# p3achyjr/p3achygo

Measured on AMD Instinct MI355X. Metric: self-play positions/sec at 1/8 MI355X, b12c256btl3 19x19 n=32, higher is better.
Workload: dtype f16; 1 GPU; b12c256btl3 random-init, self-play: C++ host (Gumbel MCTS n=32, default k<=5, selected k=5) -> p3hip_run over batches of 1024 leaf positions -> results back to the search; one step = one round = one engine batch of each of the 8 game groups = 8192 positions; batch_per_gpu=1024, concurrent_games_per_gpu=8192, game_groups_per_gpu=8, lanes_per_group=1, ladder_node_budget=0, parallelism=games sharded x1, no collective

## Files before the change

include/p3hip.h:

```cpp
#ifndef P3HIP_H_
#define P3HIP_H_

#include <stddef.h>
#include <stdint.h>

#ifdef __cplusplus
extern "C" {
#endif

#define P3HIP_BOARD_LEN 19
#define P3HIP_NUM_LOCS 361
#define P3HIP_NUM_MOVES 362
#define P3HIP_NUM_LAST_MOVES 5
#define P3HIP_NUM_VALUE_LOGITS 2
#define P3HIP_NUM_SCORE_LOGITS 800
#define P3HIP_NUM_PLANES 15
#define P3HIP_NUM_SCALARS 8

#define P3HIP_KIND_HIP 5

typedef struct p3hip_loc {
  int32_t i;
  int32_t j;
} p3hip_loc;
// ... 57 lines not shown
#define P3HIP_CONV_SET \
  "conv: C a multiple of 32 with 64 <= C <= 512; btl (1-3 inner layers) and nbt blocks with C_b a multiple of 16, " \
  "32 <= C_b <= C; classic blocks of two 3x3 convs (C_b ignored); broadcast blocks at any interval >= 2"

p3hip_engine* p3hip_create(const char* weights_path, int batch_size, int version,
                           int device_ordinal, uint32_t flags);
p3hip_engine* p3hip_create_rows(const char* weights_path, int batch_size, int version, int device_ordinal,
                                uint32_t flags, int symmetry_rows);
const char* p3hip_create_error(void);
void p3hip_destroy(p3hip_engine* e);

int p3hip_kind(const p3hip_engine* e);
const char* p3hip_path(const p3hip_engine* e);
int p3hip_batch_size(const p3hip_engine* e);

int p3hip_load_slot(p3hip_engine* e, int slot, const p3hip_features* f);
int p3hip_run(p3hip_engine* e);
int p3hip_get_slot(p3hip_engine* e, int slot, p3hip_result* out);
int p3hip_get_ownership(p3hip_engine* e, int slot, float out[P3HIP_NUM_LOCS]);
const char* p3hip_last_error(const p3hip_engine* e);

int p3hip_cache_enable(p3hip_engine* e, int log2_entries);
int p3hip_load_slot_keyed(p3hip_engine* e, int slot, const p3hip_features* f, uint64_t key_lo, uint64_t key_hi,
                          int symmetry);
int p3hip_get_slot_keyed(p3hip_engine* e, int slot, p3hip_result* out, int* symmetry, int* from_cache);
int p3hip_cache_stats(const p3hip_engine* e, uint64_t out[4]);

int p3hip_int8_calibrate(p3hip_engine* e);
int p3hip_int8_scales(const p3hip_engine* e, float* out, int n);
int p3hip_int8_set_scales(p3hip_engine* e, const float* scales, int n);

int p3hip_set_symmetries(p3hip_engine* e, uint32_t mask);
void p3hip_symmetry_maps(uint16_t fwd[8][361], uint16_t inv[8][361]);

int p3hip_set_slot_symmetries(p3hip_engine* e, int slot, uint32_t mask);
int p3hip_debug_symmetry_rows(const uint8_t* masks, int n, int rows, int* first, int* total);

#define P3HIP_AUX_LEN 837
int p3hip_get_aux(p3hip_engine* e, int slot, float out[P3HIP_AUX_LEN]);

typedef struct p3hip_labels {
  float policy[P3HIP_NUM_MOVES];
  float score_margin;
  int32_t did_win;
} p3hip_labels;
#define P3HIP_NUM_SCORE_TERMS 6
int p3hip_load_labels(p3hip_engine* e, int slot, const p3hip_labels* labels);
int p3hip_score(p3hip_engine* e, double sums[P3HIP_NUM_SCORE_TERMS], int* n_scored);
int p3hip_get_score(p3hip_engine* e, int slot, float terms[P3HIP_NUM_SCORE_TERMS]);
int p3hip_debug_score_rows(p3hip_engine* e, const float* move_probs, const float* value_probs, const float* score_probs,
                           const p3hip_labels* labels, int n, float* terms, double sums[P3HIP_NUM_SCORE_TERMS]);

typedef struct p3hip_targets {
  float policy[P3HIP_NUM_MOVES];
  float policy_aux_dist[P3HIP_NUM_MOVES];
  float own[P3HIP_NUM_LOCS];
  float mcts_value_dist[51];
  float score_margin, q6, q16, q50, q6_score, q16_score, q50_score;
  int32_t policy_aux;
  int32_t has_pi_aux_dist, has_mcts_value_dist;
} p3hip_targets;
#define P3HIP_NUM_LOSS_TERMS 19
int p3hip_load_targets(p3hip_engine* e, int slot, const p3hip_targets* targets);
int p3hip_loss(p3hip_engine* e, double sums[P3HIP_NUM_LOSS_TERMS], int* n);
int p3hip_get_loss(p3hip_engine* e, int slot, float terms[P3HIP_NUM_LOSS_TERMS]);
int p3hip_debug_loss_rows(p3hip_engine* e, const float* raw, const float* aux, const p3hip_targets* targets, int n,
                          float* terms, double sums[P3HIP_NUM_LOSS_TERMS]);


int p3hip_forward_resident(p3hip_engine* e, int n_positions);
int p3hip_upload(p3hip_engine* e);
int p3hip_sync(p3hip_engine* e);
#define P3HIP_RAW_LEN 1889
int p3hip_get_raw(p3hip_engine* e, int slot, float* out);
double p3hip_time_trunk_kernel(p3hip_engine* e, int n_positions, int iters,
                               double* flops_per_launch, const char** kernel_name);
const char* p3hip_debug_plan(const char* weights_path, uint32_t flags, int* n_q, uint64_t* digest);
int p3hip_debug_split(int npos, int kw, int cout, int n_cu, int* strips, int* tile);
long p3hip_debug_pack_sconv(const float* w, int taps, int cin, int cout, int cin_pad, int cout_pad, uint16_t* out, long n);
long p3hip_debug_pack_wconv(const float* w, int cin, int cout, int cin_pad, int cout_pad, uint16_t* out, long n);
int p3hip_debug_wconv_grid(int npos, int cout, int n_cu, int* grid, long* units, long unit, long* tile0, int* ntiles, int* cout0);
int p3hip_debug_tfm_split(int npos, int heads, int n_cu, int* parts, int* tokens);
int p3hip_debug_edge_split(int npos, int c_pad, int n_cu, int* stem, int* dense, int* heads);
int p3hip_graph_state(const p3hip_engine* e);
int p3hip_graph_stats(const p3hip_engine* e, uint64_t out[5]);
int p3hip_debug_graph_table(const int* npos, const int* total, int n, int capacity, int* action, int* evicted);
int p3hip_blockw_stamps(p3hip_engine* e, unsigned long long* out, int n);
int p3hip_debug_x(p3hip_engine* e, float* out, int n_positions);
int p3hip_debug_act_i8(p3hip_engine* e, int8_t* out, int n_positions);
int p3hip_debug_tfm(p3hip_engine* e, int which, float* out, int n_positions);
int p3hip_debug_poison(p3hip_engine* e, int byte);
const char* p3hip_debug_poison_table(void);
void p3hip_flops_per_position(const p3hip_engine* e, double* total, double* conv3x3);
void p3hip_rope_table(double* cos_out, double* sin_out);
int p3hip_rope_table_dim(int head_dim, double* cos_out, double* sin_out);

#ifdef __cplusplus
}
#endif
#endif
```

p3achygo_amd/csrc/engine.cpp:

```cpp
#include <hip/hip_runtime.h>
#include <chrono>

#include <cmath>
#include <cstdio>
#include <cstdlib>
#include <cstring>
#include <unordered_set>
#include <string>
#include <vector>

#include "engine.h"
#include "block_i8.h"
#include "conv_any.h"
#include "conv_f32.h"
#include "conv_split.h"
#include "conv_wino.h"
#include "edge_split.h"
#include "lconv_i8.h"
#include "loss.h"
#include "transformer.h"
#include "transformer_f32.h"
#include "transformer_split.h"

using namespace eng;

namespace {

thread_local std::string g_create_error;

unsigned char* upload_buffer(p3hip_engine* e) { return e->any_sym() ? e->d_sfeats : e->d_feats; }

bool upload(p3hip_engine* e, int n) {
  return e->check(hipMemcpyAsync(upload_buffer(e), e->feats_identity ? e->h_feats : e->h_feats_compact,
                                 (size_t)n * kFeatBytes, hipMemcpyHostToDevice, e->stream), "H2D features");
}

bool download(p3hip_engine* e, int n, const float* res) {
  const size_t rec = p3::kResultFloats * 4;
  return e->check(res ? hipMemcpyAsync(e->h_out, res, n * rec, hipMemcpyDeviceToHost, e->stream)
                      : hipMemcpy2DAsync(e->h_out, rec, e->d_out, p3::kOutStride * 4, rec, n, hipMemcpyDeviceToHost, e->stream),
                  "D2H results");
}

void free_cache(p3hip_engine::DeviceCache& c) {
  hipFree(c.d_tkeys); hipFree(c.d_tmeta); hipFree(c.d_tvals); hipFree(c.d_keys); hipFree(c.d_hit); hipFree(c.d_victim);
  hipFree(c.d_lists); hipFree(c.d_sym); hipFree(c.d_feats2);
  if (c.h_keys) hipHostFree(c.h_keys);
  if (c.h_hit) hipHostFree(c.h_hit);
  if (c.h_victim) hipHostFree(c.h_victim);
  if (c.h_lists) hipHostFree(c.h_lists);
  if (c.h_sym) hipHostFree(c.h_sym);
  delete[] c.h_slot_keys;
  c = p3hip_engine::DeviceCache{};
}

int read_acts(p3hip_engine* e, const _Float16* buf, size_t first, size_t n, float* out) {
  hipStreamSynchronize(e->stream);
  if (is_f32(e->trunk_path()))
    return hipMemcpy(out, (const float*)buf + first, n * 4, hipMemcpyDeviceToHost) == hipSuccess ? 0 : 2;
  std::vector<_Float16> h(n);
  if (hipMemcpy(h.data(), buf + first, n * 2, hipMemcpyDeviceToHost) != hipSuccess) return 2;
  for (size_t i = 0; i < n; ++i) out[i] = (float)h[i];
  return 0;
}

size_t act_elems(const p3hip_engine* e, size_t channels) { return (size_t)e->rows * channels * kNLoc; }
size_t x_bytes(const p3hip_engine* e) { return act_elems(e, e->wf.C) * act_bytes(e->trunk_path()); }
size_t t_bytes(const p3hip_engine* e) {
  const size_t C = e->wf.C;
  const size_t Ct = (e->wf.btype == 0 || e->wf.btype == 1) ? std::max<size_t>(C, 2 * (size_t)e->wf.Cb) : C;
  return act_elems(e, Ct) * act_bytes(e->trunk_path());
}
size_t s_bytes(const p3hip_engine* e) { return act_elems(e, e->wf.Cb) * 2; }
size_t qkv_bytes(const p3hip_engine* e) {
  return 3 * (size_t)e->rows * p3::kTfmLPad * (size_t)e->wf.model_C * act_bytes(e->trunk_path());
}
size_t hp_bytes(const p3hip_engine* e) { return (size_t)e->rows * 96 * kNLoc * 4; }
size_t pool_bytes(const p3hip_engine* e) { return (size_t)e->rows * p3::kHeadsPoolFloats * 4; }
size_t out_bytes(const p3hip_engine* e) { return (size_t)e->batch * p3::kOutStride * 4; }
size_t cout_bytes(const p3hip_engine* e) { return (size_t)e->rows * p3::kOutStride * 4; }
size_t res_bytes(const p3hip_engine* e) { return (size_t)e->batch * p3::kResultFloats * 4; }
size_t aux_bytes(const p3hip_engine* e) { return (size_t)e->rows * p3::kAuxStride * 4; }
size_t feats_bytes(const p3hip_engine* e) { return (size_t)e->rows * kFeatBytes; }
size_t slot_feats_bytes(const p3hip_engine* e) { return (size_t)e->batch * kFeatBytes; }
size_t symtab_bytes(const p3hip_engine* e) { return (size_t)e->batch * 5; }
size_t quant_bytes(const p3hip_engine* e) { return (size_t)e->plan.n_q * 4; }
size_t arena_bytes(const p3hip_engine* e) { return e->arena_bytes; }
size_t cache_entries(const p3hip_engine* e) { return (size_t)e->cache.mask + 1; }
size_t batch_words(const p3hip_engine* e) { return (size_t)e->batch * 4; }

bool poison_qkv_tokens(p3hip_engine* e, int byte) {
  const size_t eb = act_bytes(e->trunk_path()), D = (size_t)e->plan.choice.tfm_D;
  const size_t heads = (size_t)e->plan.choice.tfm_heads;
  return e->check(hipMemset2DAsync(e->d_qkv, p3::kTfmLPad * D * eb, byte, (size_t)kNLoc * D * eb, 3 * (size_t)e->rows * heads, e->stream),
                  "poison q, k, v");
}

enum class BufClass { Poisoned, State, Index, ZeroedOnce };

const char* class_name(BufClass c) {
  switch (c) {
    case BufClass::Poisoned: return "poisoned";
    case BufClass::State: return "state";
    case BufClass::Index: return "index";
    case BufClass::ZeroedOnce: return "zeroed-once";
  }
  return "";
}

struct DeviceBuffer {
  const char* name;
  void* (*ptr)(const p3hip_engine*);
  size_t (*bytes)(const p3hip_engine*);
  BufClass cls;
  const char* zero_range = "";
  bool (*poison_rest)(p3hip_engine*, int) = nullptr;
};

#define P3_BUF(member) #member, [](const p3hip_engine* e) -> void* { return (void*)e->member; }
#define P3_BYTES(expr) [](const p3hip_engine* e) -> size_t { return expr; }

const DeviceBuffer kDeviceBuffers[] = {
    {P3_BUF(d_x), x_bytes, BufClass::Poisoned},
    {P3_BUF(d_t), t_bytes, BufClass::Poisoned},
    {P3_BUF(d_u), x_bytes, BufClass::Poisoned},
    {P3_BUF(d_s), s_bytes, BufClass::Poisoned},
    {P3_BUF(d_qkv), qkv_bytes, BufClass::ZeroedOnce, "token rows 361..383 of every head of q, k and v", poison_qkv_tokens},
    {P3_BUF(d_hp), hp_bytes, BufClass::Poisoned},
    {P3_BUF(d_pool), pool_bytes, BufClass::Poisoned},
    {P3_BUF(d_cout), cout_bytes, BufClass::Poisoned},
    {P3_BUF(d_out), out_bytes, BufClass::Poisoned},
    {P3_BUF(d_res), res_bytes, BufClass::Poisoned},
    {P3_BUF(d_aux), aux_bytes, BufClass::Poisoned},
    {P3_BUF(scoring.d_terms), P3_BYTES(batch_words(e) * P3HIP_NUM_SCORE_TERMS), BufClass::Poisoned},
    {P3_BUF(scoring.d_sums), P3_BYTES(P3HIP_NUM_SCORE_TERMS * sizeof(double)), BufClass::Poisoned},
    {P3_BUF(loss.d_terms), P3_BYTES(batch_words(e) * P3HIP_NUM_LOSS_TERMS), BufClass::Poisoned},
    {P3_BUF(loss.d_sums), P3_BYTES(P3HIP_NUM_LOSS_TERMS * sizeof(double)), BufClass::Poisoned},
    {P3_BUF(d_arena), arena_bytes, BufClass::State},
    {P3_BUF(d_amax), quant_bytes, BufClass::State},
    {P3_BUF(d_ascale), quant_bytes, BufClass::State},
    {P3_BUF(cache.d_tkeys), P3_BYTES(cache_entries(e) * 16), BufClass::State},
    {P3_BUF(cache.d_tmeta), P3_BYTES(cache_entries(e) * 4), BufClass::State},
    {P3_BUF(cache.d_tvals), P3_BYTES(cache_entries(e) * p3::kOutStride * 4), BufClass::State},
    {P3_BUF(scoring.d_labels), P3_BYTES((size_t)e->batch * sizeof(p3hip_labels)), BufClass::State},
    {P3_BUF(loss.d_targets), P3_BYTES(batch_words(e) * p3::kTgtStride), BufClass::State},
    {P3_BUF(d_bw_stamps), P3_BYTES((size_t)8 * 16 * 4 * 24 * 8), BufClass::State},
#ifdef P3_DIAG
    {P3_BUF(d_stamps), P3_BYTES((size_t)p3::kStampWgs * 8 * p3::kStampSections * p3::kStampSlots * 8), BufClass::State},
    {P3_BUF(d_spans), P3_BYTES((size_t)p3::kSpanWgs * p3::kSpanSlots * 8), BufClass::State},
#else
    {"d_stamps", [](const p3hip_engine*) -> void* { return nullptr; }, P3_BYTES(0), BufClass::State},
    {"d_spans", [](const p3hip_engine*) -> void* { return nullptr; }, P3_BYTES(0), BufClass::State},
#endif
    {P3_BUF(d_feats), feats_bytes, BufClass::Index},
    {P3_BUF(d_sfeats), slot_feats_bytes, BufClass::Index},
    {P3_BUF(d_symtab), symtab_bytes, BufClass::Index},
    {P3_BUF(cache.d_keys), P3_BYTES((size_t)e->batch * sizeof(p3::CacheKey)), BufClass::Index},
    {P3_BUF(cache.d_hit), batch_words, BufClass::Index},
    {P3_BUF(cache.d_victim), batch_words, BufClass::Index},
    {P3_BUF(cache.d_lists), P3_BYTES(5 * batch_words(e)), BufClass::Index},
    {P3_BUF(cache.d_sym), batch_words, BufClass::Index},
    {P3_BUF(cache.d_feats2), slot_feats_bytes, BufClass::Index},
    {P3_BUF(scoring.d_rows), batch_words, BufClass::Index},
    {P3_BUF(loss.d_rows), batch_words, BufClass::Index},
};

#undef P3_BUF
#undef P3_BYTES

}

extern "C" {

const char* p3hip_create_error(void) { return g_create_error.c_str(); }
int p3hip_graph_state(const p3hip_engine* e) {
  return e->graph_failed ? -1 : (e->graph_exec || e->graph_table.held() > 0 ? 1 : 0);
}

int p3hip_graph_stats(const p3hip_engine* e, uint64_t out[5]) {
  for (int i = 0; i < 5; ++i) out[i] = 0;
  if (!(e->flags & (P3HIP_FLAG_LAUNCH_GRAPH | P3HIP_FLAG_LAUNCH_GRAPH_ANY))) return 1;
  if (e->graph_any()) {
    const gt::Table& t = e->graph_table;
    out[0] = (uint64_t)t.held(); out[1] = t.captures(); out[2] = t.replays(); out[3] = t.launches(); out[4] = t.evictions();
  } else {
    out[0] = e->graph_exec ? 1 : 0; out[1] = e->graph_captures; out[2] = e->graph_replays; out[3] = e->graph_launched;
  }
  return 0;
}

int p3hip_debug_graph_table(const int* npos, const int* total, int n, int capacity, int* action, int* evicted) {
  if (!npos || !total || !action || !evicted || n < 0 || capacity < gt::kMinCapacity || capacity > gt::kMaxCapacity) return 1;
  gt::Table table(capacity);
  static const char feats = 0, res = 0;
  for (int i = 0; i < n; ++i) {
    const gt::Step s = table.see(gt::Key{npos[i], total[i], &feats, &res}, i);
    action[i] = (int)s.action;
    evicted[i] = (int)s.evicted_tag;
  }
  return 0;
}

p3hip_engine* p3hip_create(const char* weights_path, int batch_size, int version,
                           int device_ordinal, uint32_t flags) {
  return p3hip_create_rows(weights_path, batch_size, version, device_ordinal, flags, 0);
}

p3hip_engine* p3hip_create_rows(const char* weights_path, int batch_size, int version,
                                int device_ordinal, uint32_t flags, int symmetry_rows) {
  g_create_error.clear();
  if (version != 1) { g_create_error = "only model version 1 (15 planes + 8 scalars) is supported"; return nullptr; }
  if (batch_size < 1 || batch_size > (1 << 16)) { g_create_error = "bad batch size"; return nullptr; }
  const bool sym = (flags & P3HIP_FLAG_SYMMETRY_AVG) != 0;
  const bool sym_slot = (flags & P3HIP_FLAG_SYMMETRY_SLOT) != 0;
  if (sym_slot && sym) {
    g_create_error = "P3HIP_FLAG_SYMMETRY_SLOT cannot be combined with P3HIP_FLAG_SYMMETRY_AVG: a slot's symmetries come "
                     "either from the engine's mask or from its own";
    return nullptr;
  }
  if (sym_slot && (flags & P3HIP_FLAG_AUX)) {
    g_create_error = "P3HIP_FLAG_AUX cannot be combined with P3HIP_FLAG_SYMMETRY_SLOT: the aux record holds tanh, absolute "
// ... 13 lines not shown
                       std::to_string(batch_size) + " .. 8 x batch size " + std::to_string(full);
      return nullptr;
    }
    if (want > (1 << 16)) {
      g_create_error = "P3HIP_FLAG_SYMMETRY_SLOT: symmetry_rows " + std::to_string(want) +
                       " exceeds the engine's row limit of 65536 (symmetry_rows 0 means 8 x batch size)";
      return nullptr;
    }
    symmetry_rows = (int)want;
  }
  if (sym && (size_t)p3::kNumSyms * batch_size > (1u << 16)) {
    g_create_error = "P3HIP_FLAG_SYMMETRY_AVG evaluates 8 copies of every slot: 8 x batch size " +
                     std::to_string(batch_size) + " exceeds the engine's row limit of 65536 (batch size at most 8192)";
    return nullptr;
  }
  if (sym && (flags & P3HIP_FLAG_AUX)) {
    g_create_error = "P3HIP_FLAG_AUX cannot be combined with P3HIP_FLAG_SYMMETRY_AVG: the aux record holds tanh, absolute "
                     "value and softmax outputs, and their average over symmetries is nothing the reference defines";
    return nullptr;
  }
  p3hip_engine* e = new p3hip_engine();
  e->path = weights_path;
  e->batch = batch_size;
  e->device = device_ordinal;
  e->flags = flags;
  e->opt = Options::from_env();
  if (e->graph_any()) {
    e->graph_table = gt::Table(e->opt.graph_cache, e->opt.graph_min_seen);
    e->graph_slots.resize((size_t)e->opt.graph_cache);
  }
  e->sym = sym;
  e->sym_slot = sym_slot;
  e->rows = sym ? p3::kNumSyms * batch_size : sym_slot ? symmetry_rows : batch_size;
  auto fail = [&](const std::string& m) {
    g_create_error = m;
    p3hip_destroy(e);
    return (p3hip_engine*)nullptr;
  };
  if (!e->wf.load(weights_path, e->err)) return fail(e->err);
  Arena ar;
  if (!build_plan(e->wf, flags, e->opt, e->plan, ar, e->err)) return fail(e->err);
  int ndev = 0;
  if (hipGetDeviceCount(&ndev) != hipSuccess || ndev <= device_ordinal)
    return fail("no HIP device " + std::to_string(device_ordinal) + " (the HIP engine has no CPU fallback)");
  if (!e->check(hipSetDevice(device_ordinal), "hipSetDevice")) return fail(e->err);
  hipDeviceProp_t prop;
  if (!e->check(hipGetDeviceProperties(&prop, device_ordinal), "hipGetDeviceProperties")) return fail(e->err);
  if (std::string(prop.gcnArchName).rfind("gfx950", 0) != 0)
    return fail(std::string("device is ") + prop.gcnArchName + ", this engine is built for gfx950 only");
  e->n_cu = prop.multiProcessorCount;
  const size_t B = batch_size;
  const bool copies = sym || sym_slot;
  const Path path = e->trunk_path();
  e->arena_bytes = ar.host.size();
  bool ok = e->check(hipStreamCreateWithFlags(&e->stream, hipStreamNonBlocking), "hipStreamCreate") &&
            e->check(hipMalloc((void**)&e->d_arena, arena_bytes(e)), "hipMalloc arena") &&
            e->check(hipMemcpyAsync(e->d_arena, ar.host.data(), ar.host.size(), hipMemcpyHostToDevice, e->stream), "upload weights") &&
            e->check(hipHostMalloc((void**)&e->h_feats, B * kFeatBytes, hipHostMallocDefault), "hipHostMalloc") &&
            e->check(hipHostMalloc((void**)&e->h_feats_compact, B * kFeatBytes, hipHostMallocDefault), "hipHostMalloc") &&
            e->check(hipHostMalloc((void**)&e->h_out, B * p3::kResultFloats * 4, hipHostMallocDefault), "hipHostMalloc") &&
            e->check(hipMalloc((void**)&e->d_res, res_bytes(e)), "hipMalloc results") &&
            e->check(hipMalloc((void**)&e->d_feats, feats_bytes(e)), "hipMalloc feats") &&
            e->check(hipMalloc((void**)&e->d_x, x_bytes(e)), "hipMalloc x") &&
            e->check(hipMalloc((void**)&e->d_t, t_bytes(e)), "hipMalloc t") &&
            e->check(hipMalloc((void**)&e->d_u, x_bytes(e)), "hipMalloc u") &&
            (e->wf.btype != 1 || path == Path::F32Conv || e->check(hipMalloc((void**)&e->d_s, s_bytes(e)), "hipMalloc s")) &&
            (!is_tfm(path) || e->check(hipMalloc((void**)&e->d_qkv, qkv_bytes(e)), "hipMalloc qkv")) &&
            e->check(hipMalloc((void**)&e->d_hp, hp_bytes(e)), "hipMalloc hp") &&
            ((path != Path::Split && path != Path::TfmSplit) ||
             e->check(hipMalloc((void**)&e->d_pool, pool_bytes(e)), "hipMalloc pooled")) &&
            e->check(hipMalloc((void**)&e->d_out, out_bytes(e)), "hipMalloc out") &&
            (!copies || (e->check(hipMalloc((void**)&e->d_sfeats, slot_feats_bytes(e)), "hipMalloc symmetry upload") &&
                         e->check(hipMalloc((void**)&e->d_cout, cout_bytes(e)), "hipMalloc copy rows"))) &&
            (!sym_slot || (e->check(hipMalloc((void**)&e->d_symtab, symtab_bytes(e)), "hipMalloc symmetry table") &&
                           e->check(hipHostMalloc((void**)&e->h_symtab, B * 5, hipHostMallocDefault), "hipHostMalloc") &&
                           e->check(hipMemsetAsync(e->d_symtab, 0, symtab_bytes(e), e->stream), "hipMemset symmetry table"))) &&
            (!(flags & P3HIP_FLAG_AUX) || (e->check(hipMalloc((void**)&e->d_aux, aux_bytes(e)), "hipMalloc aux") &&
                                           e->check(hipMemsetAsync(e->d_aux, 0, aux_bytes(e), e->stream), "hipMemset aux"))) &&
            (!is_int8(path) || (e->check(hipMalloc((void**)&e->d_amax, quant_bytes(e)), "hipMalloc amax") &&
                          e->check(hipMalloc((void**)&e->d_ascale, quant_bytes(e)), "hipMalloc scales") &&
                          e->check(hipMemsetAsync(e->d_amax, 0, quant_bytes(e), e->stream), "hipMemset amax") &&
                          e->check(hipMemsetAsync(e->d_ascale, 0, quant_bytes(e), e->stream), "hipMemset scales")));
  if (!ok) return fail(e->err);
  e->h_scale.assign(e->plan.n_q, 0.0f);
  memset(e->h_feats, 0, B * kFeatBytes);
  if (!e->check(hipMemsetAsync(e->d_feats, 0, feats_bytes(e), e->stream), "hipMemset feats") ||
      (copies && !e->check(hipMemsetAsync(e->d_sfeats, 0, slot_feats_bytes(e), e->stream), "hipMemset symmetry upload")) ||
      (copies && !e->check(hipMemsetAsync(e->d_cout, 0, cout_bytes(e), e->stream), "hipMemset copy rows")) ||
      (is_tfm(path) && !e->check(hipMemsetAsync(e->d_qkv, 0, qkv_bytes(e), e->stream), "hipMemset qkv")) ||
      !e->check(hipMemsetAsync(e->d_out, 0, out_bytes(e), e->stream), "hipMemset out") ||
      !e->check(hipStreamSynchronize(e->stream), "upload sync")) return fail(e->err);
  e->heads_args.conv_a = e->d_arena + e->plan.heads_conv_a_off;
  e->heads_args.image = e->dev<float>(e->plan.heads_image_off);
  e->heads_args.V = e->wf.V;
  e->heads_args.gbn_scale = e->dev<float>(e->plan.heads_gbn.scale_off);
  e->heads_args.gbn_shift = e->dev<float>(e->plan.heads_gbn.shift_off);
  for (int k = 0; k < kNumHeadTensors; ++k) e->heads_args.*kHeadTensors[k].arg = e->dev<float>(e->plan.head_tensor_off[k]);
  if (flags & P3HIP_FLAG_AUX) {
    e->aux_args.V = e->wf.V;
    e->aux_args.gbn_scale = e->heads_args.gbn_scale; e->aux_args.gbn_shift = e->heads_args.gbn_shift;
    e->aux_args.gd_w = e->heads_args.gd_w; e->aux_args.gd_b = e->heads_args.gd_b;
    e->aux_args.oq_embed_w = e->heads_args.oq_embed_w; e->aux_args.oq_embed_b = e->heads_args.oq_embed_b;
    for (int k = 0; k < kNumAuxTensors; ++k) e->aux_args.*kAuxTensors[k].arg = e->dev<float>(e->plan.aux_tensor_off[k]);
  }
  e->slots = p3::SlotStates((int)B);
  e->slot_sym.assign(B, 0);
  e->row_sym.assign(B, 0);
  e->slot_mask.assign(B, 1);
  e->row_mask.assign(B, 1);
  e->has_labels.assign(B, 0);
  e->has_targets.assign(B, 0);
  e->load_seq.assign(B, 0);
  e->run_load_seq.assign(B, 0);
  return e;
}

void p3hip_destroy(p3hip_engine* e) {
  if (!e) return;
  if (e->stream || e->d_arena) (void)hipSetDevice(e->device);
  if (e->stream) hipStreamSynchronize(e->stream);
  hipFree(e->d_arena); hipFree(e->d_feats); hipFree(e->d_x); hipFree(e->d_t); hipFree(e->d_u); hipFree(e->d_s);
  hipFree(e->d_hp); hipFree(e->d_pool); hipFree(e->d_out); hipFree(e->d_res); hipFree(e->d_qkv);
  hipFree(e->d_sfeats); hipFree(e->d_cout); hipFree(e->d_aux); hipFree(e->d_symtab);
  if (e->h_symtab) hipHostFree(e->h_symtab);
  hipFree(e->d_bw_stamps);
  hipFree(e->d_amax); hipFree(e->d_ascale);
  if (e->bw_mod) hipModuleUnload(e->bw_mod);
  free_cache(e->cache);
  free_scoring(e);
  free_loss(e);
  if (e->h_feats) hipHostFree(e->h_feats);
  if (e->h_feats_compact) hipHostFree(e->h_feats_compact);
  if (e->h_out) hipHostFree(e->h_out);
  for (hipEvent_t ev : e->blk_ev) hipEventDestroy(ev);
  drop_graph(e);
  if (e->stream) hipStreamDestroy(e->stream);
  delete e;
}

const char* p3hip_debug_plan(const char* weights_path, uint32_t flags, int* n_q, uint64_t* digest) {
  g_create_error.clear();
  WeightFile wf;
  Plan plan;
  Arena ar;
  std::string err;
  if (!wf.load(weights_path, err) || !build_plan(wf, flags, Options::from_env(), plan, ar, err)) {
    g_create_error = err;
    return nullptr;
  }
  uint64_t h = 0;
  bool any_q = false;
  auto fold = [&](size_t off, size_t bytes) {
    for (size_t i = 0; i < bytes; ++i) h = (h ^ ar.host[off + i]) * 1099511628211ull;
  };
  for (const BlockPlan& b : plan.blocks)
    for (const LayerPlan& lp : b.layers)
      if (lp.qidx >= 0) {
        if (!any_q) h = 14695981039346656037ull;
        any_q = true;
        fold(lp.q_off, (size_t)lp.kw * lp.kw * lp.cin * lp.cout);
        fold(lp.qs_off, (size_t)lp.cout * 4);
      }
  if (n_q) *n_q = plan.n_q;
  if (digest) *digest = h;
  return path_name(plan.choice.path);
}

int p3hip_debug_split(int npos, int kw, int cout, int n_cu, int* strips, int* tile) {
  const Options opt = Options::from_env();
  if (npos < 1 || (kw != 1 && kw != 3) || cout < 64 || cout % 64 != 0 || n_cu < 1 || !strips || !tile || opt.split_bad) return 1;
  if (opt.split_s) { *strips = opt.split_s; *tile = opt.split_t; }
  else p3::sconv_split(npos, kw, cout, n_cu, strips, tile);
  return 0;
}

int p3hip_debug_edge_split(int npos, int c_pad, int n_cu, int* stem, int* dense, int* heads) {
  if (stem) *stem = 1;
  if (dense) *dense = 1;
  if (heads) *heads = 1;
  const Options opt = Options::from_env();
  if (npos < 1 || !p3::edge_width_ok(c_pad) || n_cu < 1 || !stem || !dense || !heads || opt.edge_bad) return 1;
  if (opt.edge_s) {
    if (!p3::edge_split_valid(c_pad, opt.edge_s, opt.edge_d, opt.edge_h)) return 1;
    *stem = opt.edge_s; *dense = opt.edge_d; *heads = opt.edge_h;
  } else {
    p3::edge_split(npos, c_pad, n_cu, stem, dense, heads);
  }
  return 0;
}

int p3hip_debug_tfm_split(int npos, int heads, int n_cu, int* parts, int* tokens) {
  const Options opt = Options::from_env();
  if (npos < 1 || heads < 1 || n_cu < 1 || !parts || !tokens || opt.tfm_split_bad) return 1;
  if (opt.tfm_split_s) { *parts = opt.tfm_split_s; *tokens = opt.tfm_split_t; }
  else p3::tfm_split(npos, heads, n_cu, parts, tokens);
  return 0;
}

long p3hip_debug_pack_sconv(const float* w, int taps, int cin, int cout, int cin_pad, int cout_pad, uint16_t* out, long n) {
  std::vector<_Float16> img;
  p3::pack_sconv(img, w, taps, cin, cout, cin_pad, cout_pad);
  for (long i = 0; i < n && i < (long)img.size(); ++i) memcpy(out + i, &img[i], 2);
  return (long)img.size();
}

long p3hip_debug_pack_wconv(const float* w, int cin, int cout, int cin_pad, int cout_pad, uint16_t* out, long n) {
  std::vector<_Float16> img;
  p3::pack_wconv(img, w, cin, cout, cin_pad, cout_pad);
  for (long i = 0; i < n && i < (long)img.size(); ++i) memcpy(out + i, &img[i], 2);
  return (long)img.size();
}

int p3hip_debug_wconv_grid(int npos, int cout, int n_cu, int* grid, long* units, long unit, long* tile0, int* ntiles, int* cout0) {
  if (npos < 1 || cout < 64 || cout > p3::kWinoMaxC || cout % 64 != 0 || n_cu < 1 || !grid || !units) return 1;
  *grid = p3::wconv_grid(npos, cout, n_cu);
  *units = p3::wconv_units(npos, cout);
  if (unit < 0 || unit >= *units) return (tile0 || ntiles || cout0) ? 1 : 0;
  long t0 = 0;
  int nt = 0, c0 = 0;
  p3::wconv_unit(npos, cout, unit, &t0, &nt, &c0);
  if (tile0) *tile0 = t0;
  if (ntiles) *ntiles = nt;
  if (cout0) *cout0 = c0;
  return 0;
}

int p3hip_kind(const p3hip_engine*) { return P3HIP_KIND_HIP; }
const char* p3hip_path(const p3hip_engine* e) { return e->path.c_str(); }
int p3hip_batch_size(const p3hip_engine* e) { return e->batch; }
const char* p3hip_last_error(const p3hip_engine* e) { return e->err.c_str(); }

int p3hip_load_slot(p3hip_engine* e, int slot, const p3hip_features* f) {
  if (slot < 0 || slot >= e->batch) return 1;
  memcpy(e->h_feats + (size_t)slot * kFeatBytes, f, kFeatBytes);
  e->slot_sym[slot] = 0;
  e->slot_mask[slot] = 1;
  e->has_labels[slot] = 0;
  e->has_targets[slot] = 0;
  ++e->load_seq[slot];
  if (e->cache.on) e->cache.h_slot_keys[slot] = p3::CacheKey{0, 0, 0};
  e->slots.loaded(slot);
  return 0;
}

int p3hip_load_slot_keyed(p3hip_engine* e, int slot, const p3hip_features* f, uint64_t key_lo, uint64_t key_hi, int symmetry) {
  if (slot < 0 || slot >= e->batch) return 1;
  if (symmetry < 0 || symmetry > 7) return 1;
  memcpy(e->h_feats + (size_t)slot * kFeatBytes, f, kFeatBytes);
  e->slot_sym[slot] = (unsigned char)symmetry;
  e->slot_mask[slot] = 1;
  e->has_labels[slot] = 0;
  e->has_targets[slot] = 0;
  ++e->load_seq[slot];
  if (e->cache.on) e->cache.h_slot_keys[slot] = p3::CacheKey{key_lo, key_hi, (unsigned long long)symmetry};
  e->slots.loaded(slot);
  return 0;
// ... 554 lines not shown
```

p3achygo_amd/csrc/engine.h:

```cpp
#pragma once

#include <hip/hip_runtime.h>

#include <atomic>
#include <mutex>
#include <string>
#include <vector>

#include "../../include/p3hip.h"
#include "graph_table.h"
#include "heads_aux.h"
#include "kernels.h"
#include "plan.h"
#include "slot_state.h"
#include "symmetry.h"

namespace eng {

constexpr size_t kFeatBytes = sizeof(p3hip_features);
static_assert(sizeof(p3hip_features) == 1860, "p3hip_features layout");
static_assert(sizeof(p3hip_result) == 4 * 1892, "p3hip_result layout");

struct Pass {
  const unsigned char* feats = nullptr;
  int npos = 0;
  float* out = nullptr;
  float* res = nullptr;
  int* timed = nullptr;
};

struct GraphSlot {
  hipGraph_t graph = nullptr;
  hipGraphExec_t exec = nullptr;
};

}

struct p3hip_engine {
  std::string path, err;
  int batch = 0, device = 0;
  uint32_t flags = 0;
  eng::WeightFile wf;
  eng::Options opt;
  eng::Plan plan;
  int n_cu = 256;
  int last_npos = 0;
  hipModule_t bw_mod = nullptr;
  hipFunction_t bw_fn = nullptr;
  unsigned long long* d_bw_stamps = nullptr;
  hipStream_t stream = nullptr;
  hipGraph_t graph = nullptr;
  hipGraphExec_t graph_exec = nullptr;
  bool graph_failed = false, graph_warm = false;
  eng::Pass graph_pass;
  uint64_t graph_captures = 0, graph_replays = 0, graph_launched = 0;
  gt::Table graph_table;
  std::vector<eng::GraphSlot> graph_slots;
  long graph_seq = 0;
  bool graph_any() const { return (flags & P3HIP_FLAG_LAUNCH_GRAPH_ANY) != 0; }
  std::vector<hipEvent_t> blk_ev;

  unsigned char* d_arena = nullptr;
  size_t arena_bytes = 0;
  p3::HeadsArgs heads_args{};
  bool calibrating = false, have_scales = false;
  unsigned* d_amax = nullptr;
  float* d_ascale = nullptr;
  std::vector<float> h_scale;
  bool sym = false;
  uint32_t sym_mask = 0xFF;
  int sym_k = 8;
  int sym_syms[p3::kNumSyms] = {0, 1, 2, 3, 4, 5, 6, 7};
  int rows = 0;
  unsigned char* d_sfeats = nullptr;
  float* d_cout = nullptr;
  bool sym_slot = false;
  std::vector<unsigned char> slot_mask, row_mask;
  unsigned char *h_symtab = nullptr, *d_symtab = nullptr;
  int tab_n = 0, tab_total = 0;
  const int* tab_first() const { return reinterpret_cast<const int*>(d_symtab); }
  const unsigned char* tab_mask() const { return d_symtab + (size_t)batch * 4; }
  bool any_sym() const { return sym || sym_slot; }

  unsigned char* h_feats = nullptr;
  unsigned char* h_feats_compact = nullptr;
  unsigned char* d_feats = nullptr;
  _Float16 *d_x = nullptr, *d_t = nullptr, *d_u = nullptr;
  _Float16* d_qkv = nullptr;
#ifdef P3_DIAG
  unsigned long long* d_stamps = nullptr;
  unsigned long long* d_spans = nullptr;
  int launch_index = 0;
#endif
  _Float16* d_s = nullptr;
  float* d_hp = nullptr;
  float* d_pool = nullptr;
  float* d_aux = nullptr;
  p3::HeadsAuxArgs aux_args{};
  float* d_out = nullptr;
  float* h_out = nullptr;
  float* d_res = nullptr;
  double t_h2d = 0, t_fwd = 0, t_d2h = 0;
  long t_runs = 0;
  bool feats_identity = false;
  p3::SlotStates slots;
  int last_n = 0;
  std::vector<unsigned char> slot_sym, row_sym;

  struct DeviceCache {
    bool on = false;
    unsigned mask = 0, run = 0;
    unsigned long long* d_tkeys = nullptr;
    unsigned* d_tmeta = nullptr;
    float* d_tvals = nullptr;
    p3::CacheKey* h_slot_keys = nullptr;
    p3::CacheKey *h_keys = nullptr, *d_keys = nullptr;
    int *h_hit = nullptr, *d_hit = nullptr, *h_victim = nullptr, *d_victim = nullptr;
    int *h_lists = nullptr, *d_lists = nullptr;
    unsigned *h_sym = nullptr, *d_sym = nullptr;
    unsigned char* d_feats2 = nullptr;
    std::vector<int> out_row;
    std::vector<unsigned char> was_hit;
    unsigned long long lookups = 0, hits = 0, inserts = 0;
  } cache;
  struct Scoring {
    std::mutex mu;
    std::atomic<bool> ready{false};
    p3hip_labels *h_slot = nullptr, *h_dense = nullptr, *d_labels = nullptr;
    int *h_rows = nullptr, *d_rows = nullptr;
    float *h_terms = nullptr, *d_terms = nullptr;
    double *h_sums = nullptr, *d_sums = nullptr;
    std::vector<int> entry_of_slot;
    long scored_run = -1;
  } scoring;
  std::vector<unsigned char> has_labels;
  struct Loss {
    std::mutex mu;
    std::atomic<bool> ready{false};
    float *h_slot = nullptr, *h_dense = nullptr, *d_targets = nullptr;
    int *h_rows = nullptr, *d_rows = nullptr;
    float *h_terms = nullptr, *d_terms = nullptr;
    double *h_sums = nullptr, *d_sums = nullptr;
    std::vector<int> entry_of_slot;
    long loss_run = -1;
  } loss;
  std::vector<unsigned char> has_targets;
// ... 38 lines not shown
```

p3achygo_amd/csrc/forward.cpp:

```cpp
#include <algorithm>
#include <cstdlib>
#include <cstring>
#include <string>

#include "block_i8.h"
#include "conv_any.h"
#include "conv_f32.h"
#include "conv_split.h"
#include "conv_wino.h"
#include "edge_split.h"
#include "engine.h"
#include "lconv_conv3.h"
#include "lconv_i8.h"
#include "transformer.h"
#include "transformer_f32.h"
#include "transformer_split.h"

namespace eng {
namespace {

int grid_for(const p3hip_engine* e, int npos, int npos_per_wg) {
  int wgs = (npos + npos_per_wg - 1) / npos_per_wg;
  return wgs < e->n_cu ? wgs : e->n_cu;
}
// ... 118 lines not shown
  if (kind != 0 && kind != 1) return 0;
  int n = 1;
  while (e->opt.fuse && n < p3::kMaxFuse && first + n < blocks.size() && blocks[first + n].kind == kind) ++n;
  return n;
}

}
}

extern "C" const unsigned char p3_blockw_hsaco[];
extern "C" const unsigned char p3_blockw_hsaco_end[];

namespace eng {
namespace {

struct BlockwArgs {
  const void* x; const void* ws; const void* prm;
  int npos, nblk, nwg, pad;
  void* stamps;
  unsigned long long pad2[2];
};
static_assert(sizeof(BlockwArgs) == 64, "kernarg layout of k_blockw");

bool load_blockw(p3hip_engine* e) {
  if (e->bw_fn) return true;
  if (!e->check(hipModuleLoadData(&e->bw_mod, p3_blockw_hsaco), "hipModuleLoadData k_blockw")) return false;
  const std::string name = "k_blockw_L" + std::to_string(e->wf.inner) + (e->opt.blockw_diag ? "_diag" : "");
  if (!e->check(hipModuleGetFunction(&e->bw_fn, e->bw_mod, name.c_str()), "hipModuleGetFunction k_blockw")) return false;
  if (e->opt.blockw_diag) {
    constexpr size_t bytes = 8 * 16 * 4 * 24 * 8;
    if (!e->check(hipMalloc((void**)&e->d_bw_stamps, bytes), "hipMalloc stamps") ||
        !e->check(hipMemsetAsync(e->d_bw_stamps, 0, bytes, e->stream), "hipMemset stamps")) return false;
  }
  return true;
}

bool launch_blockw(p3hip_engine* e, const BlockwRun& run, int npos) {
  if (!load_blockw(e)) return false;
  BlockwArgs a{};
  a.x = e->d_x;
  a.ws = e->d_arena + run.stream_off;
  a.prm = e->d_arena + run.prm_off;
  a.npos = npos;
  a.nblk = run.nblk;
  a.nwg = npos < e->n_cu ? npos : e->n_cu;
  a.stamps = e->d_bw_stamps;
  size_t size = sizeof a;
  void* cfg[] = {HIP_LAUNCH_PARAM_BUFFER_POINTER, &a, HIP_LAUNCH_PARAM_BUFFER_SIZE, &size, HIP_LAUNCH_PARAM_END};
  return e->check(hipModuleLaunchKernel(e->bw_fn, a.nwg, 1, 1, 256, 1, 1, 0, e->stream, nullptr, cfg), "launch k_blockw");
}

template <class Launch>
bool timed_launch(p3hip_engine* e, int* timed, Launch&& launch) {
  const bool on = timed && 2 * *timed + 1 < (int)e->blk_ev.size();
  if (on) hipEventRecord(e->blk_ev[2 * *timed], e->stream);
  if (!launch()) return false;
  if (on) hipEventRecord(e->blk_ev[2 * (*timed)++ + 1], e->stream);
  return true;
}


hipError_t launch_conv1x1(const p3hip_engine* e, int which, const p3::Conv1x1Args& a) {
  return runs_conv_any(e->plan.choice) ? p3::launch_conv1x1_any(e->wf.C, which, a, e->n_cu, e->stream)
                                    : p3::launch_conv1x1(e->wf.C, which, a, e->n_cu, e->stream);
}

bool enqueue_stem(p3hip_engine* e, const Pass& p) {
  const Plan& pl = e->plan;
  const int C = e->wf.C;
  if (is_f32(e->trunk_path())) {
    const p3::InitF32Args a{p.feats, (float*)e->d_x, p.npos, C, e->dev<float>(pl.init_w_off), e->dev<float>(pl.game_w_off),
                            e->dev<float>(pl.game_b_off)};
    return e->check(p3::launch_init_f32(a, e->n_cu, e->stream), "launch k_init_f32");
  }
  p3::InitArgs a{};
  a.feats = p.feats; a.x = e->d_x; a.npos = p.npos;
  a.wstream = e->d_arena + pl.init_w_off; a.nms_total = pl.init_nms;
  a.game_w = e->dev<float>(pl.game_w_off); a.game_b = e->dev<float>(pl.game_b_off);
  if (e->trunk_path() == Path::Split || e->trunk_path() == Path::TfmSplit) {
    int stem = 1, dense = 1, heads = 1;
    edge_split_of(e, p.npos, &stem, &dense, &heads);
    if (stem > 1) return e->check(p3::launch_init_split(C, a, stem, e->n_cu, e->stream), "launch k_init_split");
  }
  return e->check(runs_conv_any(e->plan.choice) ? p3::launch_init_any(C, a, grid_for(e, p.npos, 1), e->stream)
                                             : p3::launch_init(C, a, grid_for(e, p.npos, 1), e->stream), "launch k_init");
}

bool enqueue_tfm_block(p3hip_engine* e, const Pass& p, const BlockPlan& bp) {
  const int d = e->wf.model_C, D = e->plan.choice.tfm_D, npos = p.npos;
  hipStream_t s = e->stream;
  const size_t per = (size_t)e->rows * p3::kTfmLPad * d;
  _Float16 *q = e->d_qkv, *k = q + per, *v = k + per, *o = e->d_t;
  p3::TfmQkvArgs a{e->d_x, q, k, v, npos, e->dev<float>(bp.tfm.rms_in), e->d_arena + bp.tfm.wqkv,
                   e->dev<float>(e->plan.rope_cos_off), e->dev<float>(e->plan.rope_sin_off)};
  int parts = 1, tokens = 64;
  if (e->trunk_path() == Path::TfmSplit) tfm_split_of(e, npos, &parts, &tokens);
  if (!e->check(p3::launch_tfm_qkv_split(d, D, a, tokens, s), "launch k_tfm_qkv")) return false;
  const p3::TfmAttnArgs b{q, k, v, o, npos, e->plan.choice.tfm_heads};
  if (!timed_launch(e, p.timed, [&] { return e->check(p3::launch_tfm_attn_split(D, b, parts, s), "launch k_tfm_attn"); }))
    return false;
  const p3::TfmFfnArgs f{o, e->d_x, npos, e->d_arena + bp.tfm.wo, e->dev<float>(bp.tfm.rms_out),
                         e->d_arena + bp.tfm.wgu, e->d_arena + bp.tfm.wdown};
  return e->check(p3::launch_tfm_ffn_split(d, f, tokens, s), "launch k_tfm_ffn");
}

bool enqueue_tfm_block_f32(p3hip_engine* e, const Pass& p, const BlockPlan& bp) {
  const int d = e->wf.model_C, D = e->plan.choice.tfm_D, npos = p.npos;
  hipStream_t s = e->stream;
  const size_t per = (size_t)e->rows * p3::kTfmLPad * d;
  float *x = (float*)e->d_x, *q = (float*)e->d_qkv, *k = q + per, *v = k + per, *o = (float*)e->d_t;
  const p3::TfmQkvF32Args a{x, q, k, v, npos, d, D, e->dev<float>(bp.tfm.rms_in), e->dev<float>(bp.tfm.wqkv),
                            e->dev<float>(e->plan.rope_cos_off), e->dev<float>(e->plan.rope_sin_off)};
  if (!e->check(p3::launch_tfm_qkv_f32(a, s), "launch k_tfm_qkv_f32")) return false;
  const p3::TfmAttnF32Args b{q, k, v, o, npos, e->plan.choice.tfm_heads};
  if (!timed_launch(e, p.timed, [&] { return e->check(p3::launch_tfm_attn_f32(D, b, s), "launch k_tfm_attn_f32"); }))
    return false;
  const p3::TfmFfnF32Args f{o, x, npos, d, e->dev<float>(bp.tfm.wo), e->dev<float>(bp.tfm.rms_out),
                            e->dev<float>(bp.tfm.wgu), e->dev<float>(bp.tfm.wdown)};
  return e->check(p3::launch_tfm_ffn_f32(f, s), "launch k_tfm_ffn_f32");
}

template <class T>
struct Regions {
  T* buf[5];
  explicit Regions(const p3hip_engine* e) {
    const size_t half = (size_t)e->rows * e->wf.Cb * kNLoc;
    T *x = (T*)e->d_x, *t = (T*)e->d_t, *u = (T*)e->d_u;
    buf[0] = x; buf[1] = t; buf[2] = t + half; buf[3] = u; buf[4] = u + half;
  }
};

template <class Args, class T>
void fill_layer(const p3hip_engine* e, Args& a, const LayerPlan& lp, const Regions<T>& r, int npos) {
  a.in = r.buf[lp.in_buf]; a.out = r.buf[lp.out_buf]; a.npos = npos;
  a.out2 = lp.out2_buf >= 0 ? reinterpret_cast<decltype(a.out2)>(r.buf[lp.out2_buf]) : nullptr;
  a.pre = lp.pre; a.act = lp.act; a.res = lp.res; a.dual = lp.dual;
  if (a.pre) { a.scale_in = e->dev<float>(lp.pre_bn.scale_off); a.shift_in = e->dev<float>(lp.pre_bn.shift_off); }
  if (a.act == 1 || a.dual) { a.scale_out = e->dev<float>(lp.out_bn.scale_off); a.shift_out = e->dev<float>(lp.out_bn.shift_off); }
}

bool launch_layer(p3hip_engine* e, const Pass& p, const LayerPlan& lp, const char* what = nullptr) {
  const LayerKernel k = layer_kernel(e, lp.kw);
  const bool conv3 = e->trunk_path() == Path::Int8Conv3;
  switch (k) {
    case LayerKernel::LconvF32: {
      p3::LConvF32Args a{};
      fill_layer(e, a, lp, Regions<float>(e), p.npos);
      a.cin = lp.cin; a.cout = lp.cout; a.w = e->dev<float>(lp.w_off);
      return e->check(p3::launch_lconv_f32(lp.kw, a, e->n_cu, e->stream), what ? what : "launch k_lconv_f32");
    }
    case LayerKernel::Sconv: {
      p3::SConvArgs a{};
      fill_layer(e, a, lp, Regions<_Float16>(e), p.npos);
      a.cin = lp.cin; a.cout = lp.cout; a.w = e->d_arena + lp.w_off;
      if (e->opt.split_s) { a.strips = e->opt.split_s; a.tile = e->opt.split_t; }
      else p3::sconv_split(a.npos, lp.kw, a.cout, e->n_cu, &a.strips, &a.tile);
      return e->check(p3::launch_sconv(lp.kw, a, e->n_cu, e->stream), what ? what : "launch k_sconv");
    }
    case LayerKernel::Wconv: {
      p3::WConvArgs a{};
      fill_layer(e, a, lp, Regions<_Float16>(e), p.npos);
      a.cin = lp.cin; a.cout = lp.cout; a.w = e->d_arena + lp.wino_off;
      return e->check(p3::launch_wconv(a, e->n_cu, e->stream), what ? what : "launch k_wconv");
    }
    case LayerKernel::LconvI8:
    case LayerKernel::LconvI8Any: {
// ... 80 lines not shown
  p3::Conv1x1Args c1{};
  c1.in = e->d_u; c1.out16 = e->d_x; c1.npos = npos;
  c1.wstream = e->d_arena + last.w_off; c1.nms_total = last.nms;
  return bp.last_fused || e->check(launch_conv1x1(e, 1, c1), "launch conv_last");
}

bool enqueue_block_i8(p3hip_engine* e, const Pass& p, const BlockPlan& bp) {
  p3::BlockI8Args a{};
  a.x = e->d_x; a.npos = p.npos; a.inner = e->wf.inner;
  a.act_scale = e->d_ascale; a.q0 = bp.layers[0].qidx;
  for (size_t j = 0; j < bp.layers.size(); ++j) {
    const LayerPlan& lp = bp.layers[j];
    a.w[j] = e->dev<int8_t>(lp.q_off); a.w_scale[j] = e->dev<float>(lp.qs_off);
    const FoldedBN& bn = j == 0 ? lp.pre_bn : bp.layers[j - 1].out_bn;
    a.scale[j] = e->dev<float>(bn.scale_off); a.shift[j] = e->dev<float>(bn.shift_off);
  }
  auto launch = [&] { return e->check(p3::launch_block_i8(e->wf.C, a, e->n_cu, e->stream), "launch k_block_i8"); };
  return timed_launch(e, p.timed, launch);
}

bool enqueue_blockw_run(p3hip_engine* e, const Pass& p, size_t bi, int* covered) {
  const int r = e->plan.blocks[bi].bw_run;
  if (r < 0) { e->err = "internal error: no k_blockw run starts at this block"; return false; }
  const BlockwRun& run = e->plan.bw_runs[r];
  *covered = run.nblk;
  return timed_launch(e, p.timed, [&] { return launch_blockw(e, run, p.npos); });
}

bool enqueue_fused_run(p3hip_engine* e, const Pass& p, size_t bi, int* covered) {
  p3::BlockArgs a;
  *covered = joined_launch(e, bi, p.npos, &a);
  if (*covered == 0) {
    *covered = fused_run(e, bi);
    a = block_args(e, bi, *covered, p.npos);
  }
#ifdef P3_DIAG
  {
    static const int which = getenv("P3DIAG_LAUNCH") ? atoi(getenv("P3DIAG_LAUNCH")) : 1;
    constexpr size_t bytes = (size_t)p3::kStampWgs * 8 * p3::kStampSections * p3::kStampSlots * 8;
    if (!e->d_stamps && hipMalloc((void**)&e->d_stamps, bytes) == hipSuccess) hipMemset(e->d_stamps, 0, bytes);
    constexpr size_t span_bytes = (size_t)p3::kSpanWgs * p3::kSpanSlots * 8;
    if (!e->d_spans && hipMalloc((void**)&e->d_spans, span_bytes) == hipSuccess) hipMemset(e->d_spans, 0, span_bytes);
    static const int which_run = getenv("P3DIAG_RUN") ? atoi(getenv("P3DIAG_RUN")) : 1;
    const int idx = (a.nruns > 1) ? 0 : which;
    a.stamp_run = (a.nruns > 1) ? which_run : 0;
    a.spans = (e->launch_index == idx) ? e->d_spans : nullptr;
    a.stamps = (e->launch_index++ == idx) ? e->d_stamps : nullptr;
  }
#endif
  const int kind = e->plan.blocks[bi].kind;
  auto launch = [&] {
    return e->check(p3::launch_block(e->wf.C, kind, e->wf.inner, e->opt.c128_wg8, a, e->n_cu, e->stream), "launch k_block");
  };
  return timed_launch(e, p.timed, launch);
}

bool enqueue_heads(p3hip_engine* e, const Pass& p) {
  const int C = e->wf.C;
  if (is_f32(e->trunk_path())) {
    p3::LConvF32Args hc{};
    hc.in = (const float*)e->d_x; hc.out = e->d_hp; hc.npos = p.npos; hc.cin = C; hc.cout = 128; hc.hp = 1;
    hc.w = e->dev<float>(e->plan.heads_w_off);
    if (!e->check(p3::launch_lconv_f32(1, hc, e->n_cu, e->stream), "launch head convs (fp32)")) return false;
  } else if (!e->plan.choice.heads_fused) {
    p3::Conv1x1Args c{};
    c.in = e->d_x; c.out32 = e->d_hp; c.npos = p.npos;
    c.wstream = e->d_arena + e->plan.heads_w_off; c.nms_total = e->plan.heads_nms;
    if (!e->check(launch_conv1x1(e, 2, c), "launch head convs")) return false;
  }
  const bool aux = (e->flags & P3HIP_FLAG_AUX) != 0;
  if (aux && e->plan.choice.heads_fused) {
    p3::Conv1x1Args c{};
    c.in = e->d_x; c.out32 = e->d_hp; c.npos = p.npos;
    c.wstream = e->d_arena + e->plan.heads_w_off; c.nms_total = e->plan.heads_nms;
    if (!e->check(launch_conv1x1(e, 2, c), "launch head convs (aux)")) return false;
  }
  p3::HeadsArgs h = e->heads_args;
  h.x = e->d_x; h.hp = e->d_hp; h.out = p.out; h.res = p.res; h.npos = p.npos;
  int hparts = 1;
  if (!e->plan.choice.heads_fused && (e->trunk_path() == Path::Split || e->trunk_path() == Path::TfmSplit)) {
    int stem = 1, dense = 1;
    edge_split_of(e, p.npos, &stem, &dense, &hparts);
  }
  if (!(e->plan.choice.heads_fused ? e->check(p3::launch_headsx(C, h, e->n_cu, e->stream), "launch k_headsx")
        : hparts > 1               ? e->check(p3::launch_heads_split(h, e->d_pool, hparts, e->stream), "launch k_heads_pool / points / softmax")
                                   : e->check(p3::launch_heads(h, p.npos, e->stream), "launch k_heads"))) return false;
  if (!aux) return true;
  p3::HeadsAuxArgs x = e->aux_args;
  x.hp = e->d_hp; x.aux = e->d_aux; x.npos = p.npos;
  return e->check(p3::launch_heads_aux(x, e->n_cu, e->stream), "launch k_heads_aux");
}

}

void tfm_split_of(const p3hip_engine* e, int npos, int* parts, int* tokens) {
  if (e->opt.tfm_split_s) { *parts = e->opt.tfm_split_s; *tokens = e->opt.tfm_split_t; }
  else p3::tfm_split(npos, e->plan.choice.tfm_heads, e->n_cu, parts, tokens);
}

void edge_split_of(const p3hip_engine* e, int npos, int* stem, int* dense, int* heads) {
  if (e->opt.edge_s) { *stem = e->opt.edge_s; *dense = e->opt.edge_d; *heads = e->opt.edge_h; }
  else p3::edge_split(npos, e->wf.C, e->n_cu, stem, dense, heads);
}

LayerKernel layer_kernel(const p3hip_engine* e, int kw) {
  const Path path = e->trunk_path();
  if (path == Path::Int8Conv3) {
    const bool any = e->plan.choice.any_width;
    if (kw == 3 && !e->calibrating) return any ? LayerKernel::LconvI8Any : LayerKernel::LconvI8;
    return any ? LayerKernel::LconvAny : LayerKernel::Lconv;
  }
  if (path == Path::Winograd3) return kw == 3 ? LayerKernel::Wconv : e->plan.choice.any_width ? LayerKernel::LconvAny : LayerKernel::Lconv;
  if (path == Path::F32Conv) return LayerKernel::LconvF32;
  if (path == Path::Split) return LayerKernel::Sconv;
  if (is_int8(path) && !e->calibrating) return path == Path::Int8Any ? LayerKernel::LconvI8Any : LayerKernel::LconvI8;
  return runs_conv_any(e->plan.choice) || path == Path::Int8Fused128 ? LayerKernel::LconvAny : LayerKernel::Lconv;
}

const char* layer_kernel_name(LayerKernel k, int kw, int cin, int cout) {
  switch (k) {
    case LayerKernel::Lconv: return cin == 192 ? "k_lconv<3,192,192>" : "k_lconv<3,64,64>";
    case LayerKernel::LconvAny: return p3::lconv_any_kernel_name(kw);
    case LayerKernel::LconvI8: return p3::lconv_i8_kernel_name(kw, cin, cout);
    case LayerKernel::LconvI8Any: return p3::lconv_i8_any_kernel_name(kw);
    case LayerKernel::LconvF32: return p3::lconv_f32_kernel_name(kw);
    case LayerKernel::Sconv: return p3::sconv_kernel_name(kw);
    case LayerKernel::Wconv: return p3::wconv_kernel_name();
  }
  return nullptr;
}

bool enqueue_forward(p3hip_engine* e, const Pass& p) {
  const Path path = e->trunk_path();
  const std::vector<BlockPlan>& blocks = e->plan.blocks;
  if (!enqueue_stem(e, p)) return false;
#ifdef P3_DIAG
  e->launch_index = 0;
#endif
  const int stop_block = e->opt.stop_block;
  e->last_npos = p.npos;
  for (size_t bi = 0; bi < blocks.size(); ++bi) {
    if (stop_block >= 0 && (int)bi >= stop_block) return true;
    const BlockPlan& bp = blocks[bi];
    int covered = 1;
    bool ok = false;
    switch (bp.kind) {
      case 5:
        ok = path == Path::TfmF32 ? enqueue_tfm_block_f32(e, p, bp) : enqueue_tfm_block(e, p, bp);
        break;
      case 3:
        ok = path == Path::F32Conv || path == Path::Split ? enqueue_broadcast_block_layers(e, p, bp) : enqueue_broadcast_block(e, p, bp);
        break;
      case 4:
        ok = is_int8_fused(path) && !e->calibrating ? enqueue_block_i8(e, p, bp) : enqueue_layerwise_block(e, p, bp);
        break;
      default:
        ok = path == Path::Blockw ? enqueue_blockw_run(e, p, bi, &covered) : enqueue_fused_run(e, p, bi, &covered);
    }
    if (!ok) return false;
    bi += covered - 1;
  }
  if (stop_block == (int)blocks.size()) return true;
  return enqueue_heads(e, p);
}

bool stage_sym_table(p3hip_engine* e, const unsigned char* masks, int n) {
  const size_t B = (size_t)e->batch;
// ... 148 lines not shown
```

p3achygo_amd/csrc/heads_dense_phase.inc:

```
  if (t < H) {
    float s = hl[L::gd_b + t];
#pragma unroll 8
    for (int k = 0; k < 2 * H; ++k) s += sc[L::gp + k] * hl[L::gd_w + k * H + t];
    sc[L::gbias + t] = s;
  } else if (t >= 64 && t < 64 + V) {
    const int o = t - 64;
    float s = hl[L::oq_embed_b + o], gm = hl[L::gamma_pre_b + o], b = hl[L::score_pre_b + o];
#pragma unroll 8
    for (int k = 0; k < 2 * H; ++k) {
      const float x = sc[L::vp + k];
      s += x * hl[L::oq_embed_w + k * V + o];
      gm += x * hl[L::gamma_pre_w + k * V + o];
      b += x * hl[L::score_pre_w + k * V + o];
    }
    sc[L::emb + o] = mish_f(s);
    sc[L::gpre + o] = mish_f(gm);
    sc[L::base + o] = b;
  } else if (t == 192) {
    float s0 = pass_b0, so = opt_pass_b;
#pragma unroll 8
    for (int k = 0; k < 2 * H; ++k) {
      s0 += sc[L::gp + k] * hl[L::pass_w + k * 2];
      so += sc[L::gp + k] * hl[L::opt_pass_w + k];
    }
    sc[L::pi + 361] = s0 - 3.0f;
    sc[L::opt + 361] = so - 3.0f;
  }
  __syncthreads();
  if (t < 14) {
    float s = hl[L::oq_out_b + t];
#pragma unroll 8
    for (int k = 0; k < V; ++k) s += sc[L::emb + k] * hl[L::oq_out_w + k * 14 + t];
    if (t < 2) sc[L::misc + t] = s;
    if (live) {
      if (t < 2) out[kOffOutcomeLogits + t] = s;
      if (t == 5) {
        out[kOffErr2] = 4.0f / (1.0f + __expf(-s));
        if (res) res[kOffErr2] = out[kOffErr2];
      }
    }
  } else if (t == 64) {
    float s = gamma_out_b;
#pragma unroll 8
    for (int k = 0; k < V; ++k) s += sc[L::gpre + k] * hl[L::gamma_out_w + k];
    if (live) out[kOffGamma] = s;
    const float sp = s > 20.0f ? s : log1pf(__expf(s));
    sc[L::misc + 2] = fminf(sp, 10.0f);
  }
```

p3achygo_amd/csrc/kernels.h:

```cpp
#pragma once
#include <hip/hip_runtime.h>
#include <stdint.h>

namespace p3 {

constexpr int kOffMoveLogits = 0;
constexpr int kOffMoveProbs = 362;
constexpr int kOffValueProbs = 724;
constexpr int kOffScoreProbs = 726;
constexpr int kOffOptProbs = 1526;
constexpr int kOffErr2 = 1888;
constexpr int kResultFloats = 1889;
constexpr int kOffOptLogits = 1889;
constexpr int kOffOutcomeLogits = 2251;
constexpr int kOffScoreLogits = 2253;
constexpr int kOffOwnership = 3053;
constexpr int kOffGamma = 3414;
constexpr int kOutStride = 3416;

constexpr int kMaxBlockLayers = 8;

constexpr int kMaxFuse = 6;
constexpr int kMaxRuns = 4, kMaxLaunchBlocks = 12;
struct BlockParams {
// ... 29 lines not shown
  int stamp_run;
  unsigned long long* spans;
#endif
};
#ifdef P3_DIAG
constexpr int kStampWgs = 8, kStampSections = 8, kStampSlots = 32, kSpanWgs = 512, kSpanSlots = 16;
#endif

struct InitArgs {
  const void* feats;
  _Float16* x;
  int npos;
  const void* wstream;
  int nms_total;
  const float* game_w;
  const float* game_b;
};

struct Conv1x1Args {
  const _Float16* in;
  _Float16* out16;
  float* out32;
  int npos;
  const void* wstream;
  int nms_total;
  const float* scale;
  const float* shift;
};

struct LConvArgs {
  const _Float16* in;
  _Float16* out;
  _Float16* out2;
  int npos;
  const void* wstream;
  int nms_total;
  int pre, act, res, dual;
  const float *scale_in, *shift_in;
  const float *scale_out, *shift_out;
  int pair_split;
};

struct BDenseArgs {
  const _Float16* t;
  _Float16* u;
  int npos;
  const void* wstream;
  int nms_total;
  const float* bias;
  const float* scale;
  const float* shift;
};

constexpr int heads_image_floats(int H, int V) {
  return 2 * H * H + 2 * H * V + 2 * H * V + (2 * H + 1) * V + V * 14 + V + V + 4 * H + 2 * H + 2 * H + H + H + H + H + H + V + V + V + 16;
}

struct HeadsArgs {
  const float* hp;
  const _Float16* x;
  const void* conv_a;
  const float* image;
  float* out;
  float* res;
  int npos;
  int V;
  const float *gbn_scale, *gbn_shift;
  const float *gd_w, *gd_b;
  const float *moves_w;
  const float *pass_w, *pass_b;
  const float *opt_moves_w;
  const float *opt_pass_w, *opt_pass_b;
  const float *oq_embed_w, *oq_embed_b;
  const float *oq_out_w, *oq_out_b;
  const float *own_w;
  const float *gamma_pre_w, *gamma_pre_b;
  const float *gamma_out_w, *gamma_out_b;
  const float *score_pre_w, *score_pre_b;
  const float *score_out_w, *score_out_b;
};

hipError_t launch_block(int C, int kind, int L, bool wg8, const BlockArgs& a, int n_cu, hipStream_t s);
int block_macro_step_bytes(int C, bool wg8);
hipError_t launch_init(int C, const InitArgs& a, int grid, hipStream_t s);
hipError_t launch_conv1x1(int C, int which, const Conv1x1Args& a, int n_cu, hipStream_t s);
hipError_t launch_bdense(int C, const BDenseArgs& a, int grid, hipStream_t s);
hipError_t launch_lconv(int kw, int cin, int cout, const LConvArgs& a, int n_cu, hipStream_t s);
hipError_t launch_heads(const HeadsArgs& a, int grid, hipStream_t s);
inline bool heads_fusable(int C, int V) { return (C == 128 || C == 256) && (V == 32 || V == 48 || V == 64); }
hipError_t launch_headsx(int C, const HeadsArgs& a, int n_cu, hipStream_t s);

constexpr int kCacheWays = 8;
struct CacheKey { unsigned long long lo, hi, sym; };
struct CacheArgs {
  const CacheKey* keys;
  int n;
  unsigned long long* tkeys;
  unsigned* tmeta;
  float* tvals;
  unsigned mask;
  unsigned run;
  int* hit;
  int* victim;
  const int* rows;
  const int* src;
  const int* idx;
  int m;
  int out_row0;
  float* out;
  unsigned* out_sym;
  const unsigned char* feats_in;
  unsigned char* feats_out;
};
hipError_t launch_cache_probe(const CacheArgs& a, hipStream_t s);
hipError_t launch_cache_gather(const CacheArgs& a, hipStream_t s);
hipError_t launch_cache_fill(const CacheArgs& a, hipStream_t s);
hipError_t launch_cache_insert(const CacheArgs& a, hipStream_t s);
const char* block_kernel_name(int C, int kind, int L);

}
```

p3achygo_amd/csrc/kernels.hip:

```cpp
#include "kernels.h"

#include <hip/hip_runtime.h>

#include "conv_core.h"
#include "conv16.h"
#include "launch_util.h"
#include "layer_kernels.h"

namespace p3 {

#ifdef P3_DIAG
#define P3_STAMP(section, k)                                                                              \
  do {                                                                                                    \
    if (a.stamps && blockIdx.x < kStampWgs && npos_done == 1 && run == a.stamp_run && (section) < kStampSections && (threadIdx.x & 63) == 0) \
      a.stamps[((blockIdx.x * 8 + (threadIdx.x >> 6)) * kStampSections + (section)) * kStampSlots + (k)] = \
          __builtin_amdgcn_s_memtime();                                                                   \
  } while (0)
#define P3_SPAN(k)                                                                        \
  do {                                                                                    \
    if (a.spans && blockIdx.x < kSpanWgs && threadIdx.x == 0 && (k) < 8) {                \
      a.spans[blockIdx.x * kSpanSlots + (k)] = __builtin_amdgcn_s_memtime();              \
      a.spans[blockIdx.x * kSpanSlots + 8 + (k)] = __builtin_amdgcn_s_memrealtime();      \
    }                                                                                     \
  } while (0)
// ... 202 lines not shown
            EpiOut16<NT> A0;
            residual_addr16<G, CB, NT>(xin, C, pos0, a.npos, 0);
            residual_load16<NT>(xin, a.x);
            activate_loaded16<G, CB, NT>(A0, xin, a.tail_scale[run], a.tail_shift[run], 0);
            residual_addr16<G, CB, NT>(xin, C, pos0, a.npos, CB);
            residual_load16<NT>(xin, a.x);
            stash16<NT>(A1, xin);
            epilogue_write16<G, CB, NT>(smem, A0, 0);
            ring_note_inflight(ring, 12);
          }
          acc16_zero<NT>(acc);
          P3_STAMP(7, 16 * half + 1);
          conv_segment16<G, CB, 1, 1, true>(ring, smem, acc);
          P3_STAMP(7, 16 * half + 2);
          if (half == 1) activate_stashed16<G, CB, NT>(A1, a.tail_scale[run], a.tail_shift[run], CB);
          lds_barrier();
          epilogue_write16<G, CB, NT>(smem, A1, 0);
          P3_STAMP(7, 16 * half + 3);
          conv_segment16<G, CB, 1, 1, true>(ring, smem, acc);
          P3_STAMP(7, 16 * half + 4);
          lds_barrier();
          epilogue_tt16<G, CB, kTtStride, NT>(smem, acc);
          bdense_stage_params(FixedW<C>{}, prm, a.dense_bias[run], a.dense_scale[run], a.dense_shift[run]);
          P3_STAMP(7, 16 * half + 5);
          bdense_passes(FixedW<C>{}, ring, smem, prm, prm + 384, prm + 384 + C, uout, pos0, half, kTtChannels);
          P3_STAMP(7, 16 * half + 6);
          if (half == 1 && run + 1 < nruns) asm volatile("s_waitcnt vmcnt(0)" ::: "memory");
          lds_barrier();
          act_zero<G>(smem);
          lds_barrier();
          P3_STAMP(7, 16 * half + 7);
        }
        blk0 += nblk;
        continue;
      }
    }
    if (tail) {
      f32x4 acc[4][NT];
      ResRegs16<NT> tr;
      P3_STAMP(7, 0);
      ring_note_inflight(ring, 24);
      acc16_zero<NT>(acc);
      P3_STAMP(7, 1);
      conv_segment16<G, CB, 1, 1>(ring, smem, acc);
      P3_STAMP(7, 2);
      lds_barrier();
      epilogue_write16<G, CB, NT>(smem, A1, 0);
      P3_STAMP(7, 4);
      conv_segment16<G, CB, 1, 1>(ring, smem, acc);
      P3_STAMP(7, 5);
      residual_addr16<G, CB, NT>(tr, C, pos0, a.npos, 0);
      epilogue_store16_mish<NT>(acc, tr, a.tout);
      P3_STAMP(7, 6);
      {
        ResRegs16<NT> xin;
        residual_addr16<G, CB, NT>(xin, C, pos0, a.npos, 0);
        residual_load16<NT>(xin, a.x);
        stash16<NT>(A1, xin);
      }
      ring_note_inflight(ring, 12);
      acc16_zero<NT>(acc);
      P3_STAMP(7, 7);
      conv_segment16<G, CB, 1, 1>(ring, smem, acc);
      P3_STAMP(7, 8);
      activate_stashed16<G, CB, NT>(A1, a.tail_scale[run], a.tail_shift[run], 0);
      lds_barrier();
      epilogue_write16<G, CB, NT>(smem, A1, 0);
      P3_STAMP(7, 10);
      conv_segment16<G, CB, 1, 1>(ring, smem, acc);
      P3_STAMP(7, 11);
      lds_barrier();
      residual_addr16<G, CB, NT>(tr, C, pos0, a.npos, CB);
      epilogue_store16_mish<NT>(acc, tr, a.tout);
      P3_STAMP(7, 12);
    }
    blk0 += nblk;
    }
    P3_SPAN(2 + npos_done < 7 ? 2 + npos_done : 6);
  }
  ring_drain();
  P3_SPAN(7);
}

template <int C, int CP = 128>
__global__ void __launch_bounds__(kWG, 2) k_init(InitArgs a) {
  init_body<CP>(a, FixedW<C>{});
}

template <int CIN, int COUT, bool PRE, int EPI>
__global__ void __launch_bounds__(kWG, 2) k_conv1x1(Conv1x1Args a) {
  constexpr int CB = CIN >= 256 ? 128 : 64;
  constexpr int CP = (COUT >= 128 && CB == 128) ? 128 : 64;
  conv1x1_body<CB, CP, PRE, EPI>(a, FixedW<CIN>{}, FixedW<COUT>{});
}

template <int KW, int CIN, int COUT, bool PRE, bool ACT, bool RES, bool DUAL = false, int NW = 8>
__global__ void __launch_bounds__(NW * 64, 2) k_lconv(LConvArgs a) {
  lconv_body<KW, PRE, ACT, RES, DUAL, NW>(a, FixedW<CIN / 64>{}, FixedW<COUT / 64>{});
}

template <int C>
__global__ void __launch_bounds__(kWG, 2) k_bdense(BDenseArgs a) {
  bdense_body(a, FixedW<C>{});
}

template <int H, int V>
struct HeadsLds {
  static constexpr int gd_w = 0;
  static constexpr int oq_embed_w = gd_w + 2 * H * H;
  static constexpr int gamma_pre_w = oq_embed_w + 2 * H * V;
  static constexpr int score_pre_w = gamma_pre_w + 2 * H * V;
  static constexpr int oq_out_w = score_pre_w + (2 * H + 1) * V;
  static constexpr int gamma_out_w = oq_out_w + V * 14;
  static constexpr int score_out_w = gamma_out_w + V;
  static constexpr int pass_w = score_out_w + V;
  static constexpr int opt_pass_w = pass_w + 4 * H;
  static constexpr int moves_w = opt_pass_w + 2 * H;
  static constexpr int opt_moves_w = moves_w + 2 * H;
  static constexpr int own_w = opt_moves_w + H;
  static constexpr int gbn_scale = own_w + H;
  static constexpr int gbn_shift = gbn_scale + H;
  static constexpr int gd_b = gbn_shift + H;
  static constexpr int oq_embed_b = gd_b + H;
  static constexpr int gamma_pre_b = oq_embed_b + V;
  static constexpr int score_pre_b = gamma_pre_b + V;
  static constexpr int oq_out_b = score_pre_b + V;
  static constexpr int n_weights = oq_out_b + 16;
  static constexpr int gp = 0, vp = gp + 2 * H, gbias = vp + 2 * H, emb = gbias + H, gpre = emb + V,
                       base = gpre + V, red = base + V, misc = red + 16, logits = misc + 4,
                       pi = logits + 800, opt = pi + 364, n_scratch = opt + 364;
  static constexpr int kGroups = 4;
  static constexpr size_t bytes = (size_t)(n_weights + kGroups * n_scratch) * 4;
};

template <int H, int V>
__global__ void __launch_bounds__(1024) k_heads(HeadsArgs a) {
  static_assert(H == 32, "head channels");
  using L = HeadsLds<H, V>;
  extern __shared__ __attribute__((aligned(16))) float hl[];
  const int tid = threadIdx.x, g = tid >> 8, t = tid & 255;
  const int wid = t >> 6, lane = t & 63;
  auto stage = [&](int off, const float* __restrict__ src, int n) {
    for (int i = tid; i < n; i += 1024) hl[off + i] = src[i];
  };
  stage(L::gd_w, a.gd_w, 2 * H * H);
  stage(L::oq_embed_w, a.oq_embed_w, 2 * H * V);
  stage(L::gamma_pre_w, a.gamma_pre_w, 2 * H * V);
  stage(L::score_pre_w, a.score_pre_w, (2 * H + 1) * V);
  stage(L::oq_out_w, a.oq_out_w, V * 14);
  stage(L::gamma_out_w, a.gamma_out_w, V);
  stage(L::score_out_w, a.score_out_w, V);
  stage(L::pass_w, a.pass_w, 4 * H);
  stage(L::opt_pass_w, a.opt_pass_w, 2 * H);
  stage(L::moves_w, a.moves_w, 2 * H);
  stage(L::opt_moves_w, a.opt_moves_w, H);
  stage(L::own_w, a.own_w, H);
  stage(L::gbn_scale, a.gbn_scale, H);
  stage(L::gbn_shift, a.gbn_shift, H);
  stage(L::gd_b, a.gd_b, H);
  stage(L::oq_embed_b, a.oq_embed_b, V);
  stage(L::gamma_pre_b, a.gamma_pre_b, V);
  stage(L::score_pre_b, a.score_pre_b, V);
  stage(L::oq_out_b, a.oq_out_b, 14);
  const float pass_b0 = a.pass_b[0], opt_pass_b = a.opt_pass_b[0], gamma_out_b = a.gamma_out_b[0],
              score_out_b = a.score_out_b[0];
  float* sc = hl + L::n_weights + g * L::n_scratch;
  const float* base = sc + L::base, * w_sp = hl + L::score_pre_w + (2 * H) * V, * w_so = hl + L::score_out_w;
  __syncthreads();

  for (int pos4 = blockIdx.x * L::kGroups; pos4 < a.npos; pos4 += gridDim.x * L::kGroups) {
    const bool live = pos4 + g < a.npos;
    const int pos = live ? pos4 + g : a.npos - 1;
    const f32x4* __restrict__ hp4 = (const f32x4*)(a.hp + (size_t)pos * 3 * H * kNLoc);
    float* __restrict__ out = a.out + (size_t)pos * kOutStride;
    float* __restrict__ res = a.res ? a.res + (size_t)pos * kResultFloats : nullptr;
    static_assert(H % 4 == 0, "channel quads");
    for (int qd = wid; qd < 2 * H / 4; qd += 4) {
      const int c = 4 * qd;
      const f32x4* src = hp4 + (size_t)(H / 4 + qd) * kNLoc;
      f32x4 v[6];
#pragma unroll
      for (int k = 0; k < 6; ++k) {
        const int i = lane + 64 * k;
        v[k] = src[i < kNLoc ? i : kNLoc - 1];
      }
      const bool is_g = c < H;
      const int ch = is_g ? c : c - H;
#pragma unroll
      for (int e = 0; e < 4; ++e) {
        const float bsc = is_g ? hl[L::gbn_scale + ch + e] : 1.0f, bsh = is_g ? hl[L::gbn_shift + ch + e] : 0.0f;
        float s = 0.0f, m = -3.0e38f;
#pragma unroll
        for (int k = 0; k < 6; ++k) {
          float x = v[k][e];
          if (is_g) x = mish_f(x * bsc + bsh);
          if (lane + 64 * k < kNLoc) {
            s += x;
            m = fmaxf(m, x);
          }
        }
        s = wave_sum(s);
        m = wave_max(m);
        if (lane == 0) {
          float* dst = sc + (is_g ? L::gp : L::vp);
          dst[ch + e] = s * (1.0f / kNLoc);
          dst[H + ch + e] = m;
        }
      }
    }
    __syncthreads();
#include "heads_dense_phase.inc"
    for (int i = t; i < kNLoc; i += 256) {
      float pi = 0.0f, po = 0.0f, ow = 0.0f;
      const int z = launder(0);
#pragma unroll
      for (int c0 = 0; c0 < H; c0 += 8) {
        float pv[8], vv[8];
#pragma unroll
        for (int u = 0; u < 2; ++u) {
          const f32x4 p4 = hp4[(size_t)(c0 / 4 + u) * kNLoc + i];
          const f32x4 v4 = hp4[(size_t)(2 * H / 4 + c0 / 4 + u) * kNLoc + i];
#pragma unroll
          for (int e = 0; e < 4; ++e) {
            pv[4 * u + e] = p4[e];
            vv[4 * u + e] = v4[e];
          }
        }
#pragma unroll
        for (int c = 0; c < 8; ++c) {
          const float p = mish_f(pv[c] + sc[L::gbias + z + c0 + c]);
          pi += p * hl[L::moves_w + z + (c0 + c) * 2];
          po += p * hl[L::opt_moves_w + z + c0 + c];
          ow += vv[c] * hl[L::own_w + z + c0 + c];
        }
      }
      sc[L::pi + i] = pi;
      sc[L::opt + i] = po;
      if (live) out[kOffOwnership + i] = tanhf(ow);
    }
    __syncthreads();
    {
      const float gam = sc[L::misc + 2];
      for (int sidx = t; sidx < 800; sidx += 256) {
#include "heads_score_bin.inc"
        sc[L::logits + sidx] = gam * s;
      }
    }
    __syncthreads();
#include "heads_softmax_phase.inc"
  }
}

template <int C, int H, int V>
struct HeadsxLds {
  using L = HeadsLds<H, V>;
  static constexpr int kGroups = 2, NS = C / 32;
  static constexpr int part = L::n_weights + kGroups * L::n_scratch;
  static constexpr int n_part = kGroups * 4 * 4 * H;
  static constexpr size_t conv_off = ((size_t)(part + n_part) * 4 + 15) / 16 * 16;
  static constexpr size_t bytes = conv_off + (size_t)6 * NS * 1024;
};

template <int C, int H, int V>
__global__ void __launch_bounds__(512, 2) k_headsx(HeadsArgs a) {
  static_assert(H == 32 && C % 32 == 0, "head channels");
  using L = HeadsLds<H, V>;
  using X = HeadsxLds<C, H, V>;
  constexpr int NS = X::NS;
  extern __shared__ __attribute__((aligned(16))) float hl[];
  const int tid = threadIdx.x, g = tid >> 8, t = tid & 255;
  const int wid = t >> 6, lane = t & 63;
  const int n = lane & 15, q = lane >> 4;
  static_assert(L::n_weights == heads_image_floats(H, V) && L::n_weights % 4 == 0, "image = HeadsLds");
  {
    const f32x4* src = (const f32x4*)a.image;
    f32x4* dst = (f32x4*)hl;
    for (int i = tid; i < L::n_weights / 4; i += 512) dst[i] = src[i];
  }
  {
    const f32x4* src = (const f32x4*)a.conv_a;
    f32x4* dst = (f32x4*)((char*)hl + X::conv_off);
    for (int i = tid; i < 6 * NS * 64; i += 512) dst[i] = src[i];
  }
  const float pass_b0 = a.pass_b[0], opt_pass_b = a.opt_pass_b[0], gamma_out_b = a.gamma_out_b[0],
              score_out_b = a.score_out_b[0];
  float* sc = hl + L::n_weights + g * L::n_scratch;
  float* part = hl + X::part + g * (4 * 4 * H);
  const char* wlds = (const char*)hl + X::conv_off + lane * 16;
  __syncthreads();

  constexpr int NTILE = (kNLoc + 15) / 16;
  constexpr int TPW = (NTILE + 3) / 4;
  for (int pos2 = blockIdx.x * X::kGroups; pos2 < a.npos; pos2 += gridDim.x * X::kGroups) {
    const bool live = pos2 + g < a.npos;
    const int pos = live ? pos2 + g : a.npos - 1;
    float* __restrict__ out = a.out + (size_t)pos * kOutStride;
    float* __restrict__ res = a.res ? a.res + (size_t)pos * kResultFloats : nullptr;
    const _Float16* __restrict__ xp = a.x + (size_t)pos * C * kNLoc;
    float bsc[2][4], bsh[2][4], ownw[2][4];
#pragma unroll
    for (int u = 0; u < 2; ++u)
#pragma unroll
      for (int i = 0; i < 4; ++i) {
        bsc[u][i] = hl[L::gbn_scale + 16 * u + 4 * q + i];
        bsh[u][i] = hl[L::gbn_shift + 16 * u + 4 * q + i];
        ownw[u][i] = hl[L::own_w + 16 * u + 4 * q + i];
      }
    float gs[2][4], gm[2][4], vs[2][4], vm[2][4];
#pragma unroll
    for (int u = 0; u < 2; ++u)
#pragma unroll
      for (int i = 0; i < 4; ++i) { gs[u][i] = 0.0f; gm[u][i] = -3.0e38f; vs[u][i] = 0.0f; vm[u][i] = -3.0e38f; }
    f32x4 P[TPW][2];
    auto xload = [&](h8 (&xb)[NS], int tile) {
      int loc = tile * 16 + n;
      if (loc >= kNLoc) loc = kNLoc - 1;
      const _Float16* src = xp + ((size_t)q * kNLoc + loc) * 8;
#pragma unroll
      for (int s_ = 0; s_ < NS; ++s_) xb[s_] = *(const h8*)(src + (size_t)s_ * 4 * kNLoc * 8);
    };
    h8 xb[2][NS];
    xload(xb[0], wid);
#pragma unroll
    for (int k = 0; k < TPW; ++k) {
      const int tile = wid + 4 * k;
      if (k + 1 < TPW) xload(xb[(k + 1) & 1], (tile + 4 < NTILE) ? tile + 4 : NTILE - 1);
      f32x4 acc[6];
#pragma unroll
      for (int ct = 0; ct < 6; ++ct) acc[ct] = f32x4{0.f, 0.f, 0.f, 0.f};
#pragma unroll
      for (int s_ = 0; s_ < NS; ++s_)
#pragma unroll
        for (int ct = 0; ct < 6; ++ct)
          acc[ct] = __builtin_amdgcn_mfma_f32_16x16x32_f16(*(const h8*)(wlds + (ct * NS + s_) * 1024), xb[k & 1][s_], acc[ct], 0, 0, 0);
      const int loc = tile * 16 + n;
      const bool ok = tile < NTILE && loc < kNLoc;
      P[k][0] = acc[0];
      P[k][1] = acc[1];
      float ow = 0.0f;
#pragma unroll
      for (int u = 0; u < 2; ++u)
#pragma unroll
        for (int i = 0; i < 4; ++i) {
          const float y = mish_f(acc[2 + u][i] * bsc[u][i] + bsh[u][i]);
          const float v = acc[4 + u][i];
          if (ok) {
            gs[u][i] += y;
            gm[u][i] = fmaxf(gm[u][i], y);
            vs[u][i] += v;
            vm[u][i] = fmaxf(vm[u][i], v);
          }
          ow += v * ownw[u][i];
        }
      ow += __shfl_xor(ow, 16);
      ow += __shfl_xor(ow, 32);
      if (ok && live && q == 0) out[kOffOwnership + loc] = tanhf(ow);
    }
#pragma unroll
    for (int u = 0; u < 2; ++u)
#pragma unroll
      for (int i = 0; i < 4; ++i) {
#pragma unroll
        for (int m = 1; m < 16; m <<= 1) {
          gs[u][i] += __shfl_xor(gs[u][i], m);
          gm[u][i] = fmaxf(gm[u][i], __shfl_xor(gm[u][i], m));
          vs[u][i] += __shfl_xor(vs[u][i], m);
          vm[u][i] = fmaxf(vm[u][i], __shfl_xor(vm[u][i], m));
        }
        if (n == 0) {
          const int ch = 16 * u + 4 * q + i;
          float* pw = part + wid * (4 * H);
          pw[ch] = gs[u][i];
          pw[H + ch] = gm[u][i];
          pw[2 * H + ch] = vs[u][i];
          pw[3 * H + ch] = vm[u][i];
        }
      }
    __syncthreads();
    if (t < 4 * H) {
      const int kind = t / H, ch = t - kind * H;
      const float p0 = part[kind * H + ch], p1 = part[4 * H + kind * H + ch], p2 = part[8 * H + kind * H + ch],
                  p3 = part[12 * H + kind * H + ch];
      float* dst = sc + ((kind < 2) ? L::gp : L::vp);
      if ((kind & 1) == 0) dst[ch] = (p0 + p1 + p2 + p3) * (1.0f / kNLoc);
      else dst[H + ch] = fmaxf(fmaxf(p0, p1), fmaxf(p2, p3));
    }
    __syncthreads();
#include "heads_dense_phase.inc"
    {
      float gb[2][4], mw[2][4], omw[2][4];
#pragma unroll
      for (int u = 0; u < 2; ++u)
#pragma unroll
        for (int i = 0; i < 4; ++i) {
          const int c = 16 * u + 4 * q + i;
          gb[u][i] = sc[L::gbias + c];
          mw[u][i] = hl[L::moves_w + c * 2];
          omw[u][i] = hl[L::opt_moves_w + c];
        }
#pragma unroll
      for (int k = 0; k < TPW; ++k) {
        const int tile = wid + 4 * k;
        float pi = 0.0f, po = 0.0f;
#pragma unroll
        for (int u = 0; u < 2; ++u)
#pragma unroll
          for (int i = 0; i < 4; ++i) {
            const float pm = mish_f(P[k][u][i] + gb[u][i]);
            pi += pm * mw[u][i];
            po += pm * omw[u][i];
          }
        pi += __shfl_xor(pi, 16);
        pi += __shfl_xor(pi, 32);
        po += __shfl_xor(po, 16);
        po += __shfl_xor(po, 32);
        const int loc = tile * 16 + n;
        if (q == 0 && tile < NTILE && loc < kNLoc) {
          sc[L::pi + loc] = pi;
          sc[L::opt + loc] = po;
        }
      }
    }
    __syncthreads();
    {
      const float gam = sc[L::misc + 2];
#pragma unroll
      for (int pr = 0; pr < 2; ++pr) {
        const int s0 = t + 512 * pr, s1 = s0 + 256;
        const f32x2 sv = {0.05f * (float)(s0 - 400) + 0.025f, 0.05f * (float)(s1 - 400) + 0.025f};
        f32x2 acc = {score_out_b, score_out_b};
        const int z = launder(0);
#pragma unroll 8
        for (int k = 0; k < V; ++k) {
          const float b = sc[L::base + z + k], w = hl[L::score_pre_w + (2 * H) * V + z + k], o = hl[L::score_out_w + z + k];
          acc = __builtin_elementwise_fma(mish_f2(__builtin_elementwise_fma(sv, f32x2{w, w}, f32x2{b, b})), f32x2{o, o}, acc);
        }
        sc[L::logits + s0] = gam * acc[0];
        if (s1 < 800) sc[L::logits + s1] = gam * acc[1];
      }
    }
    __syncthreads();
#include "heads_softmax_phase.inc"
  }
}

template <int C, int CB, int KIND, int L, int NW, bool BC>
static hipError_t launch_block_bc(const BlockArgs& a, int n_cu, hipStream_t s) {
  constexpr int NPOS = NW == 8 ? 128 / CB : 1;
  using G = Geo<NPOS, CB, 3, NW, NW == 8 ? kKMS : 2, NW == 8 ? kRingDepth : kRingDepth4>;
  constexpr size_t lds = G::ACT_BYTES + ring_bytes(CB, G::KMS, G::RD);
  static AttrOnce once;
  if (hipError_t e = ensure_lds(once, k_block<C, CB, KIND, L, NW, BC>, lds); e != hipSuccess) return e;
  const int groups = (a.npos + NPOS - 1) / NPOS, cap = NW == 8 ? n_cu : 2 * n_cu;
  hipLaunchKernelGGL((k_block<C, CB, KIND, L, NW, BC>), dim3(groups < cap ? groups : cap), dim3(NW * 64), lds, s, a);
  return hipGetLastError();
}
template <int C, int CB, int KIND, int L, int NW>
static hipError_t launch_block_t(const BlockArgs& a, int n_cu, hipStream_t s) {
  if (a.head || a.tail || a.nruns > 1) return launch_block_bc<C, CB, KIND, L, NW, true>(a, n_cu, s);
  return launch_block_bc<C, CB, KIND, L, NW, false>(a, n_cu, s);
}

int block_macro_step_bytes(int C, bool wg8) { return C == 256 ? 128 * 32 * kKMS : (wg8 ? 64 * 32 * kKMS : 64 * 32 * 2); }

hipError_t launch_block(int C, int kind, int L, bool wg8, const BlockArgs& a, int n_cu, hipStream_t s) {
  if (C == 256 && kind == 0 && L == 3) return launch_block_t<256, 128, 0, 3, 8>(a, n_cu, s);
  if (C == 256 && kind == 0 && L == 2) return launch_block_t<256, 128, 0, 2, 8>(a, n_cu, s);
  if (C == 256 && kind == 0 && L == 1) return launch_block_t<256, 128, 0, 1, 8>(a, n_cu, s);
  if (C == 256 && kind == 1) return launch_block_t<256, 128, 1, 2, 8>(a, n_cu, s);
  if (C == 128 && wg8) {
    if (kind == 0 && L == 3) return launch_block_t<128, 64, 0, 3, 8>(a, n_cu, s);
    if (kind == 0 && L == 2) return launch_block_t<128, 64, 0, 2, 8>(a, n_cu, s);
    if (kind == 0 && L == 1) return launch_block_t<128, 64, 0, 1, 8>(a, n_cu, s);
    if (kind == 1) return launch_block_t<128, 64, 1, 2, 8>(a, n_cu, s);
  }
  if (C == 128 && kind == 0 && L == 3) return launch_block_t<128, 64, 0, 3, 4>(a, n_cu, s);
  if (C == 128 && kind == 0 && L == 2) return launch_block_t<128, 64, 0, 2, 4>(a, n_cu, s);
  if (C == 128 && kind == 0 && L == 1) return launch_block_t<128, 64, 0, 1, 4>(a, n_cu, s);
  if (C == 128 && kind == 1) return launch_block_t<128, 64, 1, 2, 4>(a, n_cu, s);
  return hipErrorInvalidValue;
}

template <class K>
static hipError_t set_lds(K kernel, size_t lds) {
  return hipFuncSetAttribute((const void*)kernel, hipFuncAttributeMaxDynamicSharedMemorySize, (int)lds);
}

hipError_t launch_init(int C, const InitArgs& a, int grid, hipStream_t s) {
  using G = Geo<1, 16, 5>;
  constexpr size_t lds = G::ACT_BYTES + ring_bytes(128) + 384 * 4;
  if (C == 192) {
    constexpr size_t lds64 = G::ACT_BYTES + ring_bytes(64) + 192 * 4;
    hipLaunchKernelGGL((k_init<192, 64>), dim3(grid), dim3(kWG), lds64, s, a);
  } else if (C == 384) {
    hipLaunchKernelGGL((k_init<384>), dim3(grid), dim3(kWG), lds, s, a);
  } else if (C == 256) {
    hipLaunchKernelGGL((k_init<256>), dim3(grid), dim3(kWG), lds, s, a);
  } else if (C == 128) {
    hipLaunchKernelGGL((k_init<128>), dim3(grid), dim3(kWG), lds, s, a);
  } else {
    return hipErrorInvalidValue;
  }
  return hipGetLastError();
}

template <int CIN, int COUT, bool PRE, int EPI>
static hipError_t launch_conv1x1_t(const Conv1x1Args& a, int n_cu, hipStream_t s) {
  constexpr int CB = CIN >= 256 ? 128 : 64;
  using G = Geo<128 / CB, CB, 1>;
  constexpr int CP = (COUT >= 128 && CB == 128) ? 128 : 64;
  const int grid = conv_split_grid(a.npos, 128 / CB, (COUT + CP - 1) / CP, n_cu);
  constexpr size_t lds = G::ACT_BYTES + ring_bytes(CP);
  static AttrOnce once;
  if (hipError_t e = ensure_lds(once, k_conv1x1<CIN, COUT, PRE, EPI>, lds); e != hipSuccess) return e;
  hipLaunchKernelGGL((k_conv1x1<CIN, COUT, PRE, EPI>), dim3(grid), dim3(kWG), lds, s, a);
  return hipGetLastError();
}

hipError_t launch_conv1x1(int C, int which, const Conv1x1Args& a, int grid, hipStream_t s) {
  if (C == 192) {
    if (which == 0) return launch_conv1x1_t<192, 192, true, 0>(a, grid, s);
    if (which == 1) return launch_conv1x1_t<192, 192, false, 1>(a, grid, s);
    if (which == 2) return launch_conv1x1_t<192, 96, false, 2>(a, grid, s);
  } else if (C == 384) {
    if (which == 0) return launch_conv1x1_t<384, 384, true, 0>(a, grid, s);
    if (which == 1) return launch_conv1x1_t<384, 384, false, 1>(a, grid, s);
    if (which == 2) return launch_conv1x1_t<384, 96, false, 2>(a, grid, s);
  } else if (C == 256) {
    if (which == 0) return launch_conv1x1_t<256, 256, true, 0>(a, grid, s);
    if (which == 1) return launch_conv1x1_t<256, 256, false, 1>(a, grid, s);
    if (which == 2) return launch_conv1x1_t<256, 96, false, 2>(a, grid, s);
  } else if (C == 128) {
    if (which == 0) return launch_conv1x1_t<128, 128, true, 0>(a, grid, s);
    if (which == 1) return launch_conv1x1_t<128, 128, false, 1>(a, grid, s);
    if (which == 2) return launch_conv1x1_t<128, 96, false, 2>(a, grid, s);
  }
  return hipErrorInvalidValue;
}

template <int KW, int CIN, int COUT, bool PRE, bool ACT, bool RES, bool DUAL, int NW>
static hipError_t launch_lconv_nw(const LConvArgs& a, int n_cu, hipStream_t s) {
  constexpr int NPOS = NW == 8 ? 2 : 1;
  using G = Geo<NPOS, 64, KW, NW, (NW == 4 && KW == 3) ? 2 : kKMS>;
  const int grid = conv_split_grid(a.npos, NPOS, COUT / 64, NW == 8 ? n_cu : 2 * n_cu);
  constexpr size_t lds = G::ACT_BYTES + ring_bytes(64, G::KMS);
  static_assert(NW == 8 || 2 * lds <= 160 * 1024, "two workgroups per CU");
  static AttrOnce once;
  if (hipError_t e = ensure_lds(once, k_lconv<KW, CIN, COUT, PRE, ACT, RES, DUAL, NW>, lds); e != hipSuccess) return e;
  LConvArgs b = a;
  b.nms_total = a.nms_total * (kKMS / G::KMS);
  static const bool turns = getenv("P3HIP_NO_PAIR_TURNS") == nullptr;
  b.pair_split = (NW == 4 && turns && grid > n_cu) ? n_cu : 0;
  hipLaunchKernelGGL((k_lconv<KW, CIN, COUT, PRE, ACT, RES, DUAL, NW>), dim3(grid), dim3(NW * 64), lds, s, b);
  return hipGetLastError();
}
template <int KW, int CIN, int COUT, bool PRE, bool ACT, bool RES, bool DUAL>
static hipError_t launch_lconv_t(const LConvArgs& a, int n_cu, hipStream_t s) {
  static const bool wg8 = getenv("P3HIP_LCONV_WG8") != nullptr;
  if (wg8) return launch_lconv_nw<KW, CIN, COUT, PRE, ACT, RES, DUAL, 8>(a, n_cu, s);
  return launch_lconv_nw<KW, CIN, COUT, PRE, ACT, RES, DUAL, 4>(a, n_cu, s);
}

hipError_t launch_lconv(int kw, int cin, int cout, const LConvArgs& a, int grid, hipStream_t s) {
  const int f = (a.pre ? 8 : 0) | (a.act ? 4 : 0) | (a.res ? 2 : 0) | (a.dual ? 1 : 0);
#define P3_LCONV(KW, CIN, COUT, PRE, ACT, RES, DUAL) \
  if (kw == KW && cin == CIN && cout == COUT && f == ((PRE ? 8 : 0) | (ACT ? 4 : 0) | (RES ? 2 : 0) | (DUAL ? 1 : 0))) \
    return launch_lconv_t<KW, CIN, COUT, PRE, ACT, RES, DUAL>(a, grid, s);
  P3_LCONV(1, 384, 192, true, true, false, false)
  P3_LCONV(1, 384, 192, false, true, false, false)
  P3_LCONV(1, 384, 192, true, false, false, true)
  P3_LCONV(1, 384, 192, false, false, false, true)
  P3_LCONV(3, 192, 192, false, true, false, false)
  P3_LCONV(3, 192, 192, true, true, false, false)
  P3_LCONV(3, 192, 192, false, false, true, false)
  P3_LCONV(3, 192, 192, false, false, true, true)
  P3_LCONV(1, 192, 384, false, false, true, false)
  P3_LCONV(1, 192, 384, false, false, true, true)
  P3_LCONV(1, 256, 128, true, true, false, false)
  P3_LCONV(3, 128, 128, false, true, false, false)
  P3_LCONV(1, 128, 256, false, false, true, false)
#undef P3_LCONV
  return hipErrorInvalidValue;
}

hipError_t launch_bdense(int C, const BDenseArgs& a, int grid, hipStream_t s) {
  constexpr size_t lds = 128 * kTtStride + ring_bytes(128) + (384 + 2 * 384) * 4;
  static AttrOnce once[4];
  {
    hipError_t e = C == 256 ? ensure_lds(once[0], k_bdense<256>, lds) : C == 128 ? ensure_lds(once[1], k_bdense<128>, lds)
                 : C == 384 ? ensure_lds(once[2], k_bdense<384>, lds) : C == 192 ? ensure_lds(once[3], k_bdense<192>, lds)
                 : hipErrorInvalidValue;
    if (e != hipSuccess) return e;
  }
  if (C == 192) {
    hipLaunchKernelGGL((k_bdense<192>), dim3(grid), dim3(kWG), lds, s, a);
  } else if (C == 384) {
    hipLaunchKernelGGL((k_bdense<384>), dim3(grid), dim3(kWG), lds, s, a);
  } else if (C == 256) {
    hipLaunchKernelGGL((k_bdense<256>), dim3(grid), dim3(kWG), lds, s, a);
  } else if (C == 128) {
    hipLaunchKernelGGL((k_bdense<128>), dim3(grid), dim3(kWG), lds, s, a);
  } else {
    return hipErrorInvalidValue;
  }
  return hipGetLastError();
}

template <int V>
static hipError_t launch_heads_t(const HeadsArgs& a, hipStream_t s) {
  using L = HeadsLds<32, V>;
  static AttrOnce once;
  if (hipError_t e = ensure_lds(once, k_heads<32, V>, L::bytes); e != hipSuccess) return e;
  const int grid = (a.npos + L::kGroups - 1) / L::kGroups;
  hipLaunchKernelGGL((k_heads<32, V>), dim3(grid), dim3(1024), L::bytes, s, a);
  return hipGetLastError();
}

template <int C, int V>
static hipError_t launch_headsx_t(const HeadsArgs& a, int n_cu, hipStream_t s) {
  using X = HeadsxLds<C, 32, V>;
  static_assert(X::bytes <= 160 * 1024, "LDS");
  static AttrOnce once;
  if (hipError_t e = ensure_lds(once, k_headsx<C, 32, V>, X::bytes); e != hipSuccess) return e;
  const int groups = (a.npos + X::kGroups - 1) / X::kGroups;
  hipLaunchKernelGGL((k_headsx<C, 32, V>), dim3(groups < n_cu ? groups : n_cu), dim3(512), X::bytes, s, a);
  return hipGetLastError();
}

hipError_t launch_headsx(int C, const HeadsArgs& a, int n_cu, hipStream_t s) {
  if (C == 256 && a.V == 64) return launch_headsx_t<256, 64>(a, n_cu, s);
  if (C == 256 && a.V == 48) return launch_headsx_t<256, 48>(a, n_cu, s);
  if (C == 256 && a.V == 32) return launch_headsx_t<256, 32>(a, n_cu, s);
  if (C == 128 && a.V == 64) return launch_headsx_t<128, 64>(a, n_cu, s);
  if (C == 128 && a.V == 48) return launch_headsx_t<128, 48>(a, n_cu, s);
  if (C == 128 && a.V == 32) return launch_headsx_t<128, 32>(a, n_cu, s);
  return hipErrorInvalidValue;
}

hipError_t launch_heads(const HeadsArgs& a, int grid, hipStream_t s) {
  (void)grid;
  if (a.V == 64) return launch_heads_t<64>(a, s);
  if (a.V == 80) return launch_heads_t<80>(a, s);
  if (a.V == 48) return launch_heads_t<48>(a, s);
  if (a.V == 32) return launch_heads_t<32>(a, s);
  return hipErrorInvalidValue;
}

__global__ void __launch_bounds__(256) k_cache_probe(CacheArgs a) {
  const int r = blockIdx.x * 256 + threadIdx.x;
  if (r >= a.n) return;
  const unsigned long long lo = a.keys[r].lo, hi = a.keys[r].hi;
  int hit = -1, victim = -1;
  if (lo | hi) {
    unsigned best_age = 0;
    bool have = false;
    const unsigned h = (unsigned)(lo ^ (lo >> 32));
#pragma unroll 1
    for (int w = 0; w < kCacheWays; ++w) {
      const unsigned i = (h + (unsigned)w) & a.mask;
      const unsigned long long tl = a.tkeys[2 * (size_t)i], th = a.tkeys[2 * (size_t)i + 1];
      if (tl == lo && th == hi) { hit = (int)i; break; }
      const unsigned age = (tl | th) ? (a.run - (a.tmeta[i] >> 3)) & 0x1fffffffu : 0xffffffffu;
      if (!have || age > best_age) { have = true; best_age = age; victim = (int)i; }
    }
    if (hit >= 0) victim = -1;
  }
  a.hit[r] = hit;
  a.victim[r] = victim;
}

__global__ void __launch_bounds__(256) k_cache_gather(CacheArgs a) {
  const int j = blockIdx.x;
  const unsigned* src = (const unsigned*)(a.feats_in + (size_t)a.rows[j] * FeatOff::size);
  unsigned* dst = (unsigned*)(a.feats_out + (size_t)j * FeatOff::size);
  for (int i = threadIdx.x; i < FeatOff::size / 4; i += 256) dst[i] = src[i];
}

__global__ void __launch_bounds__(256) k_cache_fill(CacheArgs a) {
  const int j = blockIdx.x;
  const int e = a.idx[j];
  const f32x4* src = (const f32x4*)(a.tvals + (size_t)e * kOutStride);
  f32x4* dst = (f32x4*)(a.out + (size_t)(a.out_row0 + j) * kOutStride);
  static_assert(kOutStride % 4 == 0, "records are copied in 16-byte pieces");
  for (int i = threadIdx.x; i < kOutStride / 4; i += 256) dst[i] = src[i];
  if (threadIdx.x == 0) {
    const unsigned meta = a.tmeta[e];
    a.out_sym[a.out_row0 + j] = meta & 7u;
    a.tmeta[e] = (meta & 7u) | (a.run << 3);
  }
}

__global__ void __launch_bounds__(256) k_cache_insert(CacheArgs a) {
  const int j = blockIdx.x;
  const int e = a.idx[j], r = a.rows[j];
  const f32x4* src = (const f32x4*)(a.out + (size_t)a.src[j] * kOutStride);
  f32x4* dst = (f32x4*)(a.tvals + (size_t)e * kOutStride);
  for (int i = threadIdx.x; i < kOutStride / 4; i += 256) dst[i] = src[i];
  if (threadIdx.x == 0) {
    a.tkeys[2 * (size_t)e] = a.keys[r].lo;
    a.tkeys[2 * (size_t)e + 1] = a.keys[r].hi;
    a.tmeta[e] = ((unsigned)a.keys[r].sym & 7u) | (a.run << 3);
  }
}

hipError_t launch_cache_probe(const CacheArgs& a, hipStream_t s) {
  if (a.n <= 0) return hipSuccess;
  hipLaunchKernelGGL(k_cache_probe, dim3((a.n + 255) / 256), dim3(256), 0, s, a);
  return hipGetLastError();
}
hipError_t launch_cache_gather(const CacheArgs& a, hipStream_t s) {
  if (a.m <= 0) return hipSuccess;
  hipLaunchKernelGGL(k_cache_gather, dim3(a.m), dim3(256), 0, s, a);
// ... 21 lines not shown
```

p3achygo_amd/csrc/layer_kernels.h:

```cpp
#pragma once
#include "conv_core.h"
#include "kernels.h"

namespace p3 {

template <int N>
struct FixedW {
  static constexpr bool fixed = true;
  __host__ __device__ static constexpr int get() { return N; }
};
struct RuntimeW {
  static constexpr bool fixed = false;
  int n;
  __host__ __device__ int get() const { return n; }
};

struct FeatOff {
  static constexpr int color = 4, komi = 8, board = 12, last = 376, atari = 416, two = 777,
                       three = 1138, ladder = 1499, size = 1860;
};

constexpr int kTtStride = 784;
constexpr int kTtChannels = 128;
constexpr uint32_t kTtBytes = kTtChannels * kTtStride;

struct GeoTt {
  static constexpr int NW = 8, KMS = kKMS, RD = kRingDepth;
  static constexpr int NPOS = 1, CB = 384, NCH = 48, SLOTB = kTtStride, PAD = 0, S = 1, NROWS = 128,
                       NT_POS = 4, PADTOP = 0, PSLOTS = 128, ACT_BYTES = 128 * kTtStride, NT_TOTAL = 4;
};

template <class W>
__device__ __forceinline__ void bdense_passes(W wc, Ring<16384>& ring, char* smem, const float* p_bias, const float* p_scale,
                                              const float* p_shift, _Float16* __restrict__ u, int pos, int half, int nch) {
  const int C = wc.get();
  constexpr int CH = kTtChannels;
  const int lane = threadIdx.x & 63;
  const int wid = __builtin_amdgcn_readfirstlane(threadIdx.x >> 6);
  const int jg = wid & 1;
  const int ct = wid >> 1;
  const int lr = lane & 31, h = lane >> 5;
  const bool ct_active = ct * 32 < nch;
#pragma unroll 1
  for (int jp = 0; jp < 3; ++jp) {
    f32x16 acc2[2][1];
    acc_zero<GeoTt, 128>(acc2);
    conv_segment<GeoTt, 128, 1, 1, true>(ring, smem, acc2);
    if (!ct_active) continue;
#include "bdense_epilogue.inc"
  }
}

template <class W>
__device__ __forceinline__ void bdense_stage_params(W wc, float* dst, const float* __restrict__ bias,
                                                    const float* __restrict__ scale, const float* __restrict__ shift) {
  const int C = wc.get();
  for (int i = threadIdx.x; i < 384; i += kWG) dst[i] = i < kNLoc ? bias[i] : 0.0f;
  for (int i = threadIdx.x; i < C; i += kWG) { dst[384 + i] = scale[i]; dst[384 + C + i] = shift[i]; }
}

template <int CP, class W>
__device__ __forceinline__ void init_body(InitArgs a, W wc) {
  const int C = wc.get();
  using G = Geo<1, 16, 5>;
  if constexpr (W::fixed) static_assert(W::get() % CP == 0, "output passes");
  using T = Tiling<G, CP>;
  extern __shared__ __attribute__((aligned(16))) char smem[];
  constexpr uint32_t kRingOff = G::ACT_BYTES;
  act_zero<G>(smem);
  Ring<T::RS> ring;
  ring_init(ring, smem, a.wstream, a.nms_total, kRingOff);
  lds_barrier();
  const int lane = threadIdx.x & 63;
  const int wid = __builtin_amdgcn_readfirstlane(threadIdx.x >> 6);
  const int lg = wid / T::CG;
  const int lr = lane & 31, h = lane >> 5;

  for (int pos = blockIdx.x; pos < a.npos; pos += gridDim.x) {
#include "stem_planes.inc"

    float* bias_lds = (float*)(smem + kRingOff + ring_bytes(CP));
    int tc = threadIdx.x;
    if constexpr (!W::fixed) tc = launder(tc);
    if (tc < C) {
      float b = a.game_b[tc];
#pragma unroll
      for (int k = 0; k < 8; ++k) b += a.game_w[k * C + tc] * gsv[k];
      bias_lds[tc] = b;
    }

#pragma unroll 1
    for (int cp = 0; cp < C / CP; ++cp) {
      f32x16 acc[2][T::NT];
      acc_zero<G, CP>(acc);
      conv_segment<G, CP, 5, 28>(ring, smem, acc);
      const int bias_cp = cp;
#include "stem_epilogue.inc"
    }
    lds_barrier();
  }
  ring_drain();
}

template <int CB, int CP, bool PRE, int EPI, class WI, class WO>
__device__ __forceinline__ void conv1x1_body(Conv1x1Args a, WI wi, WO wo) {
  const int CIN = wi.get(), COUT = wo.get();
  constexpr int NPOS = 128 / CB;
  using G = Geo<NPOS, CB, 1>;
  using T = Tiling<G, CP>;
  const int NCP = (COUT + CP - 1) / CP;
  extern __shared__ __attribute__((aligned(16))) char smem[];
  constexpr uint32_t kRingOff = G::ACT_BYTES;
  act_zero<G>(smem);
  const int cp = (blockIdx.x >> 3) % NCP;
  const int pg0 = (blockIdx.x / (8 * NCP)) * 8 + (blockIdx.x & 7);
  const int pg_stride = gridDim.x / NCP;
  Ring<T::RS> ring;
  ring_init(ring, smem, (const char*)a.wstream + (size_t)cp * (a.nms_total / NCP) * T::RS, a.nms_total / NCP, kRingOff);
  lds_barrier();
  const int lane = threadIdx.x & 63;
  const int wid = __builtin_amdgcn_readfirstlane(threadIdx.x >> 6);
  const int lg = wid / T::CG;
  const int lr = lane & 31;

  const int NIP = CIN / CB;
  XRegs<G> xr;
  stage_load<G>(xr, a.in, CIN, pg0 * NPOS, a.npos, 0);
  int pending_stores = 0;
  for (int pos0 = pg0 * NPOS; pos0 < a.npos; pos0 += pg_stride * NPOS) {
    f32x16 acc[2][T::NT];
    acc_zero<G, CP>(acc);
#pragma unroll 1
    for (int ip = 0; ip < NIP; ++ip) {
      if (PRE) stage_math<G>(xr, ip * G::NCH, a.scale, a.shift);
      lds_barrier();
      stage_store<G, false>(smem, xr, ip * G::NCH, nullptr, nullptr);
      int nip = ip + 1, npos0 = pos0;
      if (nip == NIP) {
        nip = 0;
        npos0 = pos0 + pg_stride * NPOS;
      }
      stage_load<G>(xr, a.in, CIN, npos0, a.npos, nip * G::NCH);
      ring_note_inflight(ring, pending_stores + kXLoads);
      pending_stores = 0;
      conv_segment<G, CP, 1, 1>(ring, smem, acc);
    }
    static_assert(EPI == 2 || T::NT == 3, "vmcnt bookkeeping: 12 sixteen-byte stores per pass");
    pending_stores = (EPI == 2) ? 0 : 12;
    if (EPI == 1) {
      epilogue_to_global<G, CP, true>(acc, a.out16, COUT, pos0, a.npos, cp * CP);
    } else if (EPI == 0) {
#pragma unroll
      for (int mt = 0; mt < 2; ++mt)
#pragma unroll
        for (int j = 0; j < T::NT; ++j)
#pragma unroll
          for (int i = 0; i < 16; ++i) acc[mt][j][i] = mish_f(acc[mt][j][i]);
      epilogue_to_global<G, CP, false>(acc, a.out16, COUT, pos0, a.npos, cp * CP);
    } else {
      const int h = lane >> 5;
#pragma unroll
      for (int j = 0; j < T::NT; ++j) {
        const int t = lg + j * T::LG;
        if (t >= G::NT_TOTAL) continue;
        const int p = t / G::NT_POS, tt = t - p * G::NT_POS;
        const int loc = tt * 32 + lr;
        if (loc >= kNLoc || pos0 + p >= a.npos) continue;
        if constexpr (WO::fixed) static_assert(WO::get() % 4 == 0, "channel quads");
#pragma unroll
        for (int mt = 0; mt < 2; ++mt)
#pragma unroll
          for (int g4 = 0; g4 < 4; ++g4) {
            const int wid_cg = wid % T::CG;
            const int c0 = cp * CP + wid_cg * 64 + mt * 32 + 8 * g4 + 4 * h;
            if (c0 < COUT)
              *(f32x4*)(a.out32 + (((size_t)(pos0 + p) * (COUT / 4) + (c0 >> 2)) * kNLoc + loc) * 4) =
                  f32x4{acc[mt][j][4 * g4], acc[mt][j][4 * g4 + 1], acc[mt][j][4 * g4 + 2], acc[mt][j][4 * g4 + 3]};
          }
      }
// ... 157 lines not shown
```

p3achygo_amd/csrc/plan.cpp:

```cpp
#include "plan.h"

#include <cmath>
#include <cstdio>
#include <cstdlib>
#include <utility>

#include "../../include/p3hip.h"
#include "conv_any.h"
#include "conv_f32.h"
#include "conv_split.h"
#include "conv_wino.h"
#include "edge_split.h"
#include "graph_table.h"
#include "lconv_i8.h"
#include "transformer.h"
#include "transformer_f32.h"
#include "transformer_split.h"

namespace eng {

Options Options::from_env() {
  auto set = [](const char* n) { return getenv(n) != nullptr; };
  auto num = [](const char* n, int dflt) { return getenv(n) ? atoi(getenv(n)) : dflt; };
  Options o;
  o.c128_wg8 = set("P3HIP_C128_WG8");
  o.bcast_fuse = !set("P3HIP_NO_BFUSE");
  o.dense_fuse = !set("P3HIP_NO_DFUSE");
  o.heads_fuse = !set("P3HIP_NO_HFUSE");
  o.stop_block = num("P3HIP_DEBUG_STOP_BLOCK", -1);
  o.fuse = !set("P3HIP_NO_FUSE");
  o.join = o.fuse && !set("P3HIP_NO_JOIN");
  o.stagger = num("P3HIP_STAGGER", -1);
  o.pair_turns = !set("P3HIP_NO_PAIR_TURNS");
  o.direct_results = !set("P3HIP_NO_DIRECT_RESULTS");
  o.time_run = set("P3HIP_TIME_RUN");
  o.blockw = num("P3HIP_BLOCKW", 0) != 0;
  o.blockw_diag = set("P3HIP_BLOCKW_DIAG");
  o.conv_any = num("P3HIP_CONV_ANY", 0) != 0;
  if (const char* sp = getenv("P3HIP_SPLIT")) {
    char tail = 0;
    if (sscanf(sp, "%d,%d%c", &o.split_s, &o.split_t, &tail) != 2 || !p3::sconv_split_valid(o.split_s, o.split_t)) {
      o.split_s = o.split_t = 0;
      o.split_bad = true;
    }
  }
  if (const char* sp = getenv("P3HIP_TFM_SPLIT")) {
    char tail = 0;
    if (sscanf(sp, "%d,%d%c", &o.tfm_split_s, &o.tfm_split_t, &tail) != 2 || !p3::tfm_split_valid(o.tfm_split_s, o.tfm_split_t)) {
      o.tfm_split_s = o.tfm_split_t = 0;
      o.tfm_split_bad = true;
    }
  }
  if (const char* sp = getenv("P3HIP_EDGE_SPLIT")) {
    char tail = 0;
    if (strcmp(sp, "0") == 0) {
      o.edge_s = o.edge_d = o.edge_h = 1;
    } else if (sscanf(sp, "%d,%d,%d%c", &o.edge_s, &o.edge_d, &o.edge_h, &tail) != 3 || o.edge_s < 1 || o.edge_s > 8 ||
               !p3::edge_split_valid(64, 1, o.edge_d, o.edge_h)) {
      o.edge_s = o.edge_d = o.edge_h = 0;
      o.edge_bad = true;
    }
  }
  o.graph_cache = gt::capacity_from(getenv("P3HIP_GRAPH_CACHE"));
  if (o.graph_cache == 0) {
    o.graph_cache = gt::kDefaultCapacity;
    o.graph_cache_bad = true;
  }
  o.graph_min_seen = std::min(std::max(num("P3HIP_GRAPH_MIN_SEEN", gt::kMinSeen), gt::kMinSeen), 64);
  o.graph_max_rows = std::max(num("P3HIP_GRAPH_MAX_ROWS", gt::kDefaultMaxRows), 0);
  return o;
}

const char* path_name(Path p) {
  switch (p) {
    case Path::Refused: return "Refused";
    case Path::Fused: return "Fused";
    case Path::Blockw: return "Blockw";
    case Path::Layerwise: return "Layerwise";
    case Path::ConvAny: return "ConvAny";
    case Path::Int8: return "Int8";
    case Path::Int8Fused256: return "Int8Fused256";
    case Path::Int8Fused128: return "Int8Fused128";
    case Path::Int8Any: return "Int8Any";
    case Path::Int8Conv3: return "Int8Conv3";
    case Path::Winograd3: return "Winograd3";
    case Path::F32Conv: return "F32Conv";
    case Path::Split: return "Split";
    case Path::Tfm: return "Tfm";
    case Path::TfmF32: return "TfmF32";
    case Path::TfmSplit: return "TfmSplit";
  }
  return "?";
}

namespace {

enum class Trunk {
  None,
  BlockShape,
  LconvShape,
  OtherConv,
  Transformer,
};

struct TrunkClass {
  Trunk trunk = Trunk::None;
  bool tfm_file = false;
  bool btl123 = false;
  bool in_set = false;
  bool hv_ok = false;
  bool classic = false;
// ... 126 lines not shown
}

PlanChoice choose_plan(const WeightFile& wf, uint32_t flags, const Options& opt, std::string& err) {
  const int C = wf.C, Cb = wf.Cb;
  PlanChoice c;
  const TrunkClass t = classify(wf);
  const Request r = read_request(flags, t, C, opt);
  const Request::Kind k = r.kind;
  const Trunk tr = t.trunk;
  const struct { bool applies; std::string text; } refusals[] = {
      {k == Request::LowLatency && t.tfm_file && !r.ll_tfm,
       "P3HIP_FLAG_LOW_LATENCY serves the conv trunks (" P3HIP_CONV_SET "); the transformer trunks (" P3HIP_TRANSFORMER_SET
       ") have no low-latency plan"},
      {k == Request::LowLatencyTfm && !t.tfm_file,
       "P3HIP_FLAG_LOW_LATENCY_TFM serves the transformer trunks only (" P3HIP_TRANSFORMER_SET "); the conv trunks have "
       "P3HIP_FLAG_LOW_LATENCY"},
      {k == Request::Winograd && t.tfm_file,
       "P3HIP_FLAG_WINOGRAD serves the conv trunks (" P3HIP_CONV_SET ") whose fp16 plan runs layer by layer; the "
       "transformer trunks (" P3HIP_TRANSFORMER_SET ") have no 3x3 convs"},
      {r.int8_conv3 && t.tfm_file,
       "P3HIP_FLAG_INT8_CONV3 serves the conv trunks (" P3HIP_CONV_SET ") whose fp16 plan runs layer by layer; the "
       "transformer trunks (" P3HIP_TRANSFORMER_SET ") have no INT8 plan"},
      {r.int8_any && t.tfm_file,
       "P3HIP_FLAG_INT8_ANY serves the conv trunks (" P3HIP_CONV_SET "); the transformer trunks (" P3HIP_TRANSFORMER_SET
       ") have no INT8 plan"},
      {k == Request::Fp32 && t.tfm_file && !r.f32_tfm,
       "P3HIP_FLAG_FP32 serves the conv trunks only (" P3HIP_CONV_SET "); the transformer trunks run in fp16, or in "
       "fp32 with P3HIP_FLAG_FP32_TFM"},
      {k == Request::Fp32 && !t.tfm_file && !r.f32_conv,
       "P3HIP_FLAG_FP32_TFM serves the transformer trunks only (" P3HIP_TRANSFORMER_SET "); the conv trunks have "
       "P3HIP_FLAG_FP32"},
      {!r.clash.empty(), r.clash},
      {(flags & P3HIP_FLAG_LAUNCH_GRAPH_ANY) && opt.graph_cache_bad,
       "P3HIP_FLAG_LAUNCH_GRAPH_ANY: P3HIP_GRAPH_CACHE must be a whole number of graphs from 1 to 1024 (default 64)"},
      {k == Request::LowLatency && !t.tfm_file && opt.split_bad,
       "P3HIP_FLAG_LOW_LATENCY: P3HIP_SPLIT must be \"S,T\" with S row strips of 1, 2 or 4 and output tiles of T = 16, 32 "
       "or 64 channels"},
      {(k == Request::LowLatencyTfm || (k == Request::LowLatency && t.tfm_file)) && opt.tfm_split_bad,
       "P3HIP_FLAG_LOW_LATENCY_TFM: P3HIP_TFM_SPLIT must be \"S,T\" with S query parts of 1, 2, 3 or 6 and T = 16, 32 or 64 "
       "tokens per workgroup"},
      {(k == Request::LowLatency || k == Request::LowLatencyTfm) &&
           (opt.edge_bad || (opt.edge_s && !p3::edge_split_valid(C, opt.edge_s, opt.edge_d, opt.edge_h))),
       "P3HIP_FLAG_LOW_LATENCY / P3HIP_FLAG_LOW_LATENCY_TFM: P3HIP_EDGE_SPLIT must be \"0\" or \"s,d,h\" with s = 1 or the "
       "stem's output passes (the stream's channels / 128, or / 64 where they are no multiple of 128), d = 1, 3 or 12 parts "
       "of the broadcast dense and h = 1, 4 or 8 parts of the heads"},
      {tr == Trunk::None || (k == Request::Int8Any && tr == Trunk::BlockShape && !t.in_set) || !t.hv_ok,
       "unsupported architecture for the HIP engine (need a conv trunk (" P3HIP_CONV_SET "), or a transformer "
       "trunk (" P3HIP_TRANSFORMER_SET "); H=32, V in {32,48,64,80} (transformer: V in {32,48,64}, and 80 at "
       "d > 256))"},
      {k == Request::Winograd && tr == Trunk::BlockShape,
       "P3HIP_FLAG_WINOGRAD serves the trunks whose fp16 plan runs layer by layer; the C = 256 / C_b = 128 and C = 128 / "
       "C_b = 64 btl and nbt trunks run the fused block kernel, and a layer-wise Winograd plan for them is not built"},
      {r.int8_conv3 && tr == Trunk::BlockShape,
       "P3HIP_FLAG_INT8_CONV3 serves the trunks whose fp16 plan runs layer by layer; the C = 256 / C_b = 128 and C = 128 / "
       "C_b = 64 btl and nbt trunks run the fused block kernel, which no layer-wise plan approaches: P3HIP_FLAG_INT8_FUSED, "
       "P3HIP_FLAG_INT8_C128 and P3HIP_FLAG_INT8_ANY serve them"},
      {k == Request::Int8C128 && !(r.alone && tr == Trunk::BlockShape && C == 128 && t.btl123),
       "INT8_C128 is available only for C = 128 / C_b = 64 trunks of btl blocks with 1, 2 or 3 inner layers "
       "(b12c128btl3, b10c128btl3, small and their kin, broadcast blocks at any interval), and not together with "
       "another INT8 flag; nbt trunks, the other widths (P3HIP_FLAG_INT8_FUSED serves C = 256 / C_b = 128 btl trunks, "
       "P3HIP_FLAG_INT8 the layer-wise trunks) and the transformer are not served"},
      {(k == Request::Int8 || k == Request::Int8Fused) && tr == Trunk::OtherConv,
       std::string(k == Request::Int8Fused ? "INT8_FUSED" : "INT8") + " is not available for this conv trunk: "
       "P3HIP_FLAG_INT8 serves C = 384 / C_b = 192 btl or nbt blocks and C = 192 classic blocks, P3HIP_FLAG_INT8_FUSED "
       "serves C = 256 / C_b = 128 btl blocks with 1, 2 or 3 inner layers, P3HIP_FLAG_INT8_C128 serves C = 128 / "
       "C_b = 64 btl blocks with 1, 2 or 3 inner layers; the other widths run in fp16 only"},
      {k == Request::Int8Fused && !(r.alone && tr == Trunk::BlockShape && C == 256 && t.btl123),
       "INT8_FUSED is available only for C = 256 / C_b = 128 trunks of btl blocks with 1, 2 or 3 inner layers "
       "(b12c256btl3 and its kin, broadcast blocks at any interval), and not together with P3HIP_FLAG_INT8; nbt and "
       "C = 128 trunks, the layer-wise trunks (P3HIP_FLAG_INT8 serves those) and the transformer are not served"},
      {k == Request::Int8 && tr != Trunk::LconvShape,
       "INT8 is available only for layer-wise trunks (C = 384 / C_b = 192 btl or nbt blocks, C = 192 classic "
       "blocks); this trunk runs fused block kernels or the transformer"},
  };
  for (const auto& refusal : refusals)
    if (refusal.applies) {
      err = refusal.text;
      return c;
    }
  c.path = path_of(r, t, wf, opt);
  c.any_width = (c.path == Path::Int8Conv3 || c.path == Path::Winograd3) && (tr == Trunk::OtherConv || opt.conv_any);
  c.CB = is_layerwise(c.path) ? p3::conv_any_slice(C) : (is_tfm(c.path) ? 128 : Cb);
  c.CPI = is_layerwise(c.path) ? p3::conv_any_init_pass(C) : 128;
  c.heads_image = !is_f32(c.path) && p3::heads_fusable(C, wf.V);
  c.heads_fused = c.heads_image && opt.heads_fuse && !runs_conv_any(c);
  if (is_tfm(c.path)) {
    c.tfm_heads = Cb;
    c.tfm_D = wf.model_C / Cb;
  }
  return c;
}

const HeadTensor kHeadTensors[kNumHeadTensors] = {
    {"policy.gpool_dense.w", &p3::HeadsArgs::gd_w, 2 * 32 * 32, 0, 0},
    {"policy.gpool_dense.b", &p3::HeadsArgs::gd_b, 32, 0, 12},
    {"policy.out_moves.w", &p3::HeadsArgs::moves_w, 2 * 32, 0, 9},
    {"policy.out_pass.w", &p3::HeadsArgs::pass_w, 4 * 32, 0, 7},
    {"policy.out_pass.b", &p3::HeadsArgs::pass_b, 2, 0, -1},
    {"policy.opt_moves.w", &p3::HeadsArgs::opt_moves_w, 32, 0, 10},
    {"policy.opt_pass.w", &p3::HeadsArgs::opt_pass_w, 2 * 32, 0, 8},
    {"policy.opt_pass.b", &p3::HeadsArgs::opt_pass_b, 1, 0, -1},
    {"value.oq_embed.w", &p3::HeadsArgs::oq_embed_w, 0, 2 * 32, 1},
    {"value.oq_embed.b", &p3::HeadsArgs::oq_embed_b, 0, 1, 13},
    {"value.oq_out.w", &p3::HeadsArgs::oq_out_w, 0, 14, 4},
    {"value.oq_out.b", &p3::HeadsArgs::oq_out_b, 14, 0, 16},
    {"value.own.w", &p3::HeadsArgs::own_w, 32, 0, 11},
    {"value.gamma_pre.w", &p3::HeadsArgs::gamma_pre_w, 0, 2 * 32, 2},
    {"value.gamma_pre.b", &p3::HeadsArgs::gamma_pre_b, 0, 1, 14},
    {"value.gamma_out.w", &p3::HeadsArgs::gamma_out_w, 0, 1, 5},
    {"value.gamma_out.b", &p3::HeadsArgs::gamma_out_b, 1, 0, -1},
    {"value.score_pre.w", &p3::HeadsArgs::score_pre_w, 0, 2 * 32 + 1, 3},
    {"value.score_pre.b", &p3::HeadsArgs::score_pre_b, 0, 1, 15},
    {"value.score_out.w", &p3::HeadsArgs::score_out_w, 0, 1, 6},
    {"value.score_out.b", &p3::HeadsArgs::score_out_b, 1, 0, -1}};

const AuxTensor kAuxTensors[kNumAuxTensors] = {
    {"policy.soft_moves.w", &p3::HeadsAuxArgs::soft_moves_w, 32, 0, 0, 0, {}},
    {"policy.soft_pass.w", &p3::HeadsAuxArgs::soft_pass_w, 2 * 32, 0, 0, 0, {}},
    {"policy.soft_pass.b", &p3::HeadsAuxArgs::soft_pass_b, 1, 0, 0, 0, {}},
    {"value.mcts_dist.w", &p3::HeadsAuxArgs::mcts_w, 0, p3::kAuxBins, 0, 0, {}},
    {"value.mcts_dist.b", &p3::HeadsAuxArgs::mcts_b, p3::kAuxBins, 0, 0, 0, {}},
    {"policy.out_moves.w", &p3::HeadsAuxArgs::moves_aux_w, 2 * 32, 0, 2, 1, {1}},
    {"policy.out_pass.w", &p3::HeadsAuxArgs::pass_aux_w, 4 * 32, 0, 2, 1, {1}},
    {"policy.out_pass.b", &p3::HeadsAuxArgs::pass_aux_b, 2, 0, 2, 1, {1}},
    {"value.oq_out.w", &p3::HeadsAuxArgs::oq_aux_w, 0, 14, 14, p3::kAuxGoCols, {2, 3, 4, 6, 7, 8, 9, 10, 11, 12, 13}},
    {"value.oq_out.b", &p3::HeadsAuxArgs::oq_aux_b, 14, 0, 14, p3::kAuxGoCols, {2, 3, 4, 6, 7, 8, 9, 10, 11, 12, 13}}};

namespace {

constexpr float kBnEps = 1e-3f;

void pack_segment(std::vector<_Float16>& dst, const float* W, int taps, int ntaps_pad,
                  int cin_total, int cout_total, int cin0, int CB, int cout0, int CP) {
  for (int tap = 0; tap < ntaps_pad; ++tap)
    for (int q = 0; q < CB / 16; ++q)
      for (int h = 0; h < 2; ++h)
        for (int co = 0; co < CP; ++co)
          for (int e = 0; e < 8; ++e) {
            int ci = cin0 + q * 16 + h * 8 + e, c = cout0 + co;
            float v = 0.0f;
            if (tap < taps && ci < cin_total && c < cout_total)
              v = W[((size_t)tap * cin_total + ci) * cout_total + c];
            dst.push_back((_Float16)v);
          }
}

void pack_segment_3x3(std::vector<_Float16>& dst, const float* W, int cin_total, int cout_total, int CB, int CP) {
  for (int ky = 0; ky < 3; ++ky)
    for (int q32 = 0; q32 < CB / 32; ++q32)
      for (int kx = 0; kx < 3; ++kx)
        for (int q = 2 * q32; q < 2 * q32 + 2; ++q)
          for (int h = 0; h < 2; ++h)
            for (int co = 0; co < CP; ++co)
              for (int e = 0; e < 8; ++e) {
                const int ci = q * 16 + h * 8 + e, tap = ky * 3 + kx;
                float v = 0.0f;
                if (ci < cin_total && co < cout_total) v = W[((size_t)tap * cin_total + ci) * cout_total + co];
                dst.push_back((_Float16)v);
              }
}

void pack_granule(std::vector<_Float16>& dst, const float* W, int cin_total, int cout_total, int tap, int k0, int cout0,
                  const float* scale) {
  for (int j = 0; j < 2; ++j)
    for (int c = 0; c < 2; ++c)
      for (int h = 0; h < 2; ++h)
        for (int n = 0; n < 32; ++n)
          for (int el = 0; el < 8; ++el) {
// ... 378 lines not shown
  }
  plan.heads_gbn = fold_bn(ar, wf, "policy.gpool_bn", 32);
  const float* data[kNumHeadTensors];
  size_t size[kNumHeadTensors];
  for (int k = 0; k < kNumHeadTensors; ++k) {
    size[k] = (size_t)kHeadTensors[k].n0 + (size_t)kHeadTensors[k].nV * wf.V;
    const Tensor& t = wf.get(kHeadTensors[k].name, size[k]);
    data[k] = t.data;
    plan.head_tensor_off[k] = ar.add(t.data, t.size() * 4);
  }
  if (plan.choice.heads_image && wf.missing.empty()) {
    std::vector<float> img;
    for (int rank = 0; rank <= 16; ++rank) {
      for (int k = 0; k < kNumHeadTensors; ++k)
        if (kHeadTensors[k].image_rank == rank) img.insert(img.end(), data[k], data[k] + size[k]);
      if (rank == 11)
        for (size_t off : {plan.heads_gbn.scale_off, plan.heads_gbn.shift_off}) {
          const float* bn = reinterpret_cast<const float*>(ar.host.data() + off);
          img.insert(img.end(), bn, bn + 32);
        }
    }
    img.insert(img.end(), 2, 0.0f);
    if ((int)img.size() != p3::heads_image_floats(32, wf.V)) {
      err = "internal error: heads image size";
      return false;
    }
    plan.heads_image_off = ar.add(img.data(), img.size() * 4);
  }
  return true;
}

void pack_aux(Builder& b) {
  const WeightFile& wf = b.wf;
  for (int k = 0; k < kNumAuxTensors; ++k) {
    const AuxTensor& at = kAuxTensors[k];
    const size_t n = (size_t)at.n0 + (size_t)at.nV * wf.V;
    const Tensor& t = wf.get(at.name, n);
    if (at.cols == 0) {
      b.plan.aux_tensor_off[k] = b.ar.add(t.data, n * 4);
      continue;
    }
    std::vector<float> w;
    for (size_t r = 0; r < n / at.cols; ++r)
      for (int c = 0; c < at.ntake; ++c) w.push_back(t.data[r * at.cols + at.take[c]]);
    b.plan.aux_tensor_off[k] = b.ar.add(w.data(), w.size() * 4);
  }
}

void pack_wino(Builder& b) {
  for (size_t i = 0; i < b.plan.blocks.size(); ++i) {
    BlockPlan& bp = b.plan.blocks[i];
    if (bp.kind != 4) continue;
    for (size_t j = 0; j < bp.layers.size(); ++j) {
      LayerPlan& lp = bp.layers[j];
      if (lp.kw != 3) continue;
      std::vector<_Float16> img;
      p3::pack_wconv(img, conv_w(b.wf, (int)i, (int)j, 3, lp.cin, lp.cout), lp.cin, lp.cout, lp.cin, lp.cout);
      lp.wino_off = b.ar.add(img.data(), img.size() * 2);
    }
  }
}

}

void spiral_rope_table(int D, double* cos_out, double* sin_out) {
  const int K = 4, per = D / K, nth = D / 4;
  const double kPi = 3.14159265358979323846;
  std::vector<double> theta(D);
  for (int i = 0; i < D; ++i) {
    const int k = i / per, r = (i % per) / 2;
    int t = 2 * (k % (K / 2)) + (r / 2) * K + (r % 2);
    if (t > nth - 1) t = nth - 1;
    theta[i] = std::pow(100.0, -(double)t / nth);
  }
  for (int s = 0; s < kNLoc; ++s)
    for (int i = 0; i < D; ++i) {
      const double ang = (i / per) * (kPi / K);
      const double proj = (s / 19) * std::cos(ang) + (s % 19) * std::sin(ang);
      cos_out[s * D + i] = std::cos(theta[i] * proj);
      sin_out[s * D + i] = std::sin(theta[i] * proj);
    }
}

bool build_plan(const WeightFile& wf, uint32_t flags, const Options& opt, Plan& plan, Arena& ar, std::string& err) {
  plan.choice = choose_plan(wf, flags, opt, err);
  const Path path = plan.choice.path;
  if (path == Path::Refused) return false;
  Builder b{wf, opt, plan, ar};
  pack_stem(b);
  if (is_tfm(path)) pack_rope(b);
  for (int i = 0; i < wf.nblocks; ++i) {
    if (path == Path::Tfm || path == Path::TfmSplit) pack_tfm_block<_Float16>(b, i, pack_afrag);
    else if (path == Path::TfmF32) pack_tfm_block<float>(b, i, p3::pack_tfm_f32);
    else {
      if (is_layerwise(path)) b.flush_run();
      if (wf.is_broadcast(i)) pack_broadcast_block(b, i);
      else if (is_layerwise(path)) pack_layerwise_block(b, i);
      else pack_fused_block(b, i);
    }
  }
  b.flush_run();
  lay_out_runs(b);
  if (path == Path::Blockw) pack_blockw_runs(b);
  if (!pack_heads(b, err)) return false;
  if (flags & P3HIP_FLAG_AUX) pack_aux(b);
  if (path == Path::Winograd3) pack_wino(b);
  if (!wf.missing.empty()) {
    err = "weight file lacks tensors of the architecture its header names: " + wf.missing;
    return false;
  }
  if (ar.bad_stream) {
    err = "internal error: a packed weight stream is not a whole number of ring macro-steps";
    return false;
  }
  return true;
}

}
```

p3achygo_amd/csrc/plan.h:

```cpp
#pragma once

#include <cstdint>
#include <cstring>
#include <string>
#include <vector>

#include "graph_table.h"
#include "heads_aux.h"
#include "kernels.h"
#include "weights.h"

namespace eng {

constexpr int kNLoc = 361;

struct Options {
  bool c128_wg8 = false;
  bool bcast_fuse = true;
  bool dense_fuse = true;
  bool heads_fuse = true;
  int stop_block = -1;
  bool fuse = true, join = true;
  int stagger = -1;
  bool pair_turns = true;
  bool direct_results = true;
  bool time_run = false;
  bool blockw = false;
  bool blockw_diag = false;
  bool conv_any = false;
  int split_s = 0, split_t = 0;
  bool split_bad = false;
  int tfm_split_s = 0, tfm_split_t = 0;
  bool tfm_split_bad = false;
  int edge_s = 0, edge_d = 0, edge_h = 0;
  bool edge_bad = false;
  int graph_cache = 64;
  bool graph_cache_bad = false;
  int graph_min_seen = gt::kMinSeen, graph_max_rows = gt::kDefaultMaxRows;
  static Options from_env();
};

enum class Path {
  Refused,
  Fused,
  Blockw,
  Layerwise,
  ConvAny,
  Int8,
  Int8Fused256,
  Int8Fused128,
  Int8Any,
  Int8Conv3,
  Winograd3,
  F32Conv,
  Split,
  Tfm,
  TfmF32,
  TfmSplit,
};
inline bool is_tfm(Path p) { return p == Path::Tfm || p == Path::TfmF32 || p == Path::TfmSplit; }
inline bool is_f32(Path p) { return p == Path::F32Conv || p == Path::TfmF32; }
inline bool is_int8_fused(Path p) { return p == Path::Int8Fused256 || p == Path::Int8Fused128; }
inline bool is_int8(Path p) { return p == Path::Int8 || p == Path::Int8Any || p == Path::Int8Conv3 || is_int8_fused(p); }
inline bool is_layerwise(Path p) {
  return p == Path::Layerwise || p == Path::ConvAny || is_int8(p) || p == Path::Winograd3 || p == Path::F32Conv || p == Path::Split;
}
inline size_t act_bytes(Path p) { return is_f32(p) ? 4 : 2; }

struct PlanChoice {
  Path path = Path::Refused;
  int CB = 0;
  int CPI = 0;
  bool heads_image = false;
  bool heads_fused = false;
  int tfm_heads = 0, tfm_D = 0;
  bool any_width = false;
};
inline bool runs_conv_any(const PlanChoice& c) {
  return c.path == Path::ConvAny || c.path == Path::Int8Any || c.path == Path::Split ||
         ((c.path == Path::Int8Conv3 || c.path == Path::Winograd3) && c.any_width);
}

const char* path_name(Path p);

PlanChoice choose_plan(const WeightFile& wf, uint32_t flags, const Options& opt, std::string& err);

struct Arena {
  std::vector<unsigned char> host;
  bool bad_stream = false;
  size_t add(const void* p, size_t bytes) {
    size_t off = (host.size() + 255) & ~size_t(255);
    host.resize(off + bytes);
    memcpy(host.data() + off, p, bytes);
    return off;
  }
};

struct FoldedBN { size_t scale_off, shift_off; };

struct LayerPlan {
  int kw, cin, cout;
  bool pre;
  int act;
  bool res, dual;
  FoldedBN pre_bn, out_bn;
  int in_buf, out_buf, out2_buf;
  size_t w_off = 0;
  int nms = 0;
  size_t q_off = 0, qs_off = 0;
  int qidx = -1;
  size_t wino_off = 0;
  int out_qidx = -1;
};

struct TfmPlan { size_t rms_in = 0, rms_out = 0, wqkv = 0, wo = 0, wgu = 0, wdown = 0; };

struct BlockPlan {
  int kind;
  TfmPlan tfm;
  std::vector<LayerPlan> layers;
  size_t stream_off = 0;
  int nms = 0;
  size_t stream_bytes = 0;
  FoldedBN bn[p3::kMaxBlockLayers];
  size_t dense_off = 0;
  int dense_nms = 0;
  size_t dense_bias_off = 0;
  bool first_fused = false, last_fused = false;
  bool dense_fused = false;
  int head_of = -1, tail_of = -1;
  size_t head_bytes = 0, tail_bytes = 0;
  int bw_run = -1;
};

struct HeadTensor {
  const char* name;
  const float* p3::HeadsArgs::*arg;
  int n0, nV;
  int image_rank;
};
constexpr int kNumHeadTensors = 21;
extern const HeadTensor kHeadTensors[kNumHeadTensors];

struct AuxTensor {
  const char* name;
  const float* p3::HeadsAuxArgs::*arg;
  int n0, nV;
  int cols;
  int ntake;
  int take[p3::kAuxGoCols];
};
constexpr int kNumAuxTensors = 10;
extern const AuxTensor kAuxTensors[kNumAuxTensors];

struct BlockwRun { size_t first; int nblk; size_t stream_off, prm_off; };

struct Plan {
  PlanChoice choice;
  std::vector<BlockPlan> blocks;
  size_t init_w_off = 0; int init_nms = 0;
  size_t game_w_off = 0, game_b_off = 0;
  size_t rope_cos_off = 0, rope_sin_off = 0;
  int n_q = 0;
  std::vector<BlockwRun> bw_runs;
  size_t heads_w_off = 0; int heads_nms = 0;
  size_t heads_conv_a_off = 0, heads_image_off = 0;
  FoldedBN heads_gbn{};
  size_t head_tensor_off[kNumHeadTensors] = {};
  size_t aux_tensor_off[kNumAuxTensors] = {};
};

bool build_plan(const WeightFile& wf, uint32_t flags, const Options& opt, Plan& plan, Arena& ar, std::string& err);

void spiral_rope_table(int D, double* cos_out, double* sin_out);

}
```

p3achygo_amd/csrc/stem_planes.inc:

```
  const unsigned char* f = (const unsigned char*)a.feats + (size_t)pos * FeatOff::size;
  const int color = (signed char)f[FeatOff::color];
  for (int loc = threadIdx.x; loc < kNLoc; loc += kWG) {
    h8 lo = {0, 0, 0, 0, 0, 0, 0, 0}, hi = {0, 0, 0, 0, 0, 0, 0, 0};
    auto our = [&](int off) {
      return (_Float16)((signed char)f[off + loc] == color ? 1.0f : 0.0f);
    };
    auto opp = [&](int off) {
      return (_Float16)((signed char)f[off + loc] == -color ? 1.0f : 0.0f);
    };
    lo[0] = our(FeatOff::board); lo[1] = opp(FeatOff::board);
    lo[7] = our(FeatOff::atari); hi[0] = opp(FeatOff::atari);
    hi[1] = our(FeatOff::two); hi[2] = opp(FeatOff::two);
    hi[3] = our(FeatOff::three); hi[4] = opp(FeatOff::three);
    hi[5] = our(FeatOff::ladder); hi[6] = opp(FeatOff::ladder);
    const int y = (loc * 3450) >> 16, xx = loc - y * kBL;
#pragma unroll
    for (int m = 0; m < 5; ++m) {
      const int* lm = (const int*)(f + FeatOff::last + m * 8);
      if (lm[0] == y && lm[1] == xx) lo[2 + m] = (_Float16)1.0f;
    }
    const int s = G::PADTOP + y * G::S + xx;
    *(h8*)(smem + s * G::SLOTB) = lo;
    *(h8*)(smem + s * G::SLOTB + 16) = hi;
  }
  float gsv[8];
  gsv[0] = color == 1 ? 1.0f : 0.0f;
  gsv[1] = color == 1 ? 0.0f : 1.0f;
#pragma unroll
  for (int m = 0; m < 5; ++m) {
    const int* lm = (const int*)(f + FeatOff::last + m * 8);
    gsv[2 + m] = (lm[0] == 19 && lm[1] == 0) ? 1.0f : 0.0f;
  }
  gsv[7] = (color == 1 ? -1.0f : 1.0f) * (*(const float*)(f + FeatOff::komi)) / 15.0f;
```

p3achygo_amd/engine.py:

```python
from __future__ import annotations

import ctypes as C
import enum
import os

import numpy as np

from .features import NUM_MOVES, RAW_LEN, Features, Result

_HERE = os.path.dirname(os.path.abspath(__file__))
LIB_PATH = os.environ.get("P3HIP_LIB") or os.path.join(_HERE, "csrc", "libp3hip.so")

EXPORTS = [
    "p3hip_create", "p3hip_create_error", "p3hip_destroy", "p3hip_kind", "p3hip_path",
    "p3hip_batch_size", "p3hip_load_slot", "p3hip_run", "p3hip_get_slot", "p3hip_get_ownership",
    "p3hip_last_error", "p3hip_forward_resident", "p3hip_upload", "p3hip_sync", "p3hip_get_raw",
    "p3hip_time_trunk_kernel", "p3hip_flops_per_position", "p3hip_graph_state",
    "p3hip_cache_enable", "p3hip_load_slot_keyed", "p3hip_get_slot_keyed", "p3hip_cache_stats",
    "p3hip_blockw_stamps", "p3hip_debug_x", "p3hip_debug_tfm", "p3hip_rope_table", "p3hip_rope_table_dim",
    "p3hip_int8_calibrate", "p3hip_int8_scales", "p3hip_int8_set_scales",
    "p3hip_set_symmetries", "p3hip_symmetry_maps",
    "p3hip_create_rows", "p3hip_set_slot_symmetries", "p3hip_debug_symmetry_rows",
    "p3hip_load_labels", "p3hip_score", "p3hip_get_score", "p3hip_debug_score_rows",
    "p3hip_get_aux",
    "p3hip_load_targets", "p3hip_loss", "p3hip_get_loss", "p3hip_debug_loss_rows",
    "p3hip_debug_plan", "p3hip_debug_act_i8",
    "p3hip_debug_split", "p3hip_debug_pack_sconv", "p3hip_debug_tfm_split", "p3hip_debug_edge_split",
    "p3hip_debug_poison", "p3hip_debug_poison_table",
    "p3hip_debug_pack_wconv", "p3hip_debug_wconv_grid",
    "p3hip_graph_stats", "p3hip_debug_graph_table",
]

FLAG_RUN_ALL_SLOTS = 2
FLAG_SHARED_DEVICE = 4
FLAG_LAUNCH_GRAPH = 8
FLAG_LAUNCH_GRAPH_ANY = 131072
GRAPH_STATS = ("held", "captures", "replays", "launched", "evictions")
FLAG_INT8 = 16
FLAG_INT8_FUSED = 64
FLAG_INT8_C128 = 128
FLAG_INT8_ANY = 2048
FLAG_INT8_CONV3 = 32768
FLAG_WINOGRAD = 65536
FLAG_FP32 = 256
FLAG_FP32_TFM = 512
FLAG_FP32_ANY = FLAG_FP32 | FLAG_FP32_TFM
NUM_SCORE_TERMS = 6
SCORE_TERMS = ("policy_loss", "outcome_loss", "policy_hit", "outcome_hit", "score_diff", "score_pred")
FLAG_AUX = 1024
AUX_LEN = 837
AUX_SEGMENTS = {
    "08:pi_logits_aux": (0, 362), "21:pi_logits_soft": (362, 724),
    "09:q6": (724, 725), "10:q16": (725, 726), "11:q50": (726, 727),
    "13:q16_err": (727, 728), "14:q50_err": (728, 729),
    "15:q6_score": (729, 730), "16:q16_score": (730, 731), "17:q50_score": (731, 732),
    "18:q6_score_err": (732, 733), "19:q16_score_err": (733, 734), "20:q50_score_err": (734, 735),
    "23:mcts_dist_logits": (735, 786), "24:mcts_dist_probs": (786, 837),
}
RAW_SEGMENTS = {
    "00:pi_logits": (0, 362), "22:pi_logits_optimistic": (362, 724), "02:outcome_logits": (724, 726),
    "05:score_logits": (726, 1526), "04:own": (1526, 1887), "12:q6_err": (1887, 1888), "07:gamma": (1888, 1889),
}
RESULT_FIELDS = {"01:pi": "move_probs", "03:outcome": "value_probs", "06:score_probs": "score_probs"}
OUTPUT_NAMES = tuple(sorted(list(AUX_SEGMENTS) + list(RAW_SEGMENTS) + list(RESULT_FIELDS)))
FLAG_LOW_LATENCY = 4096
FLAG_LOW_LATENCY_TFM = 8192
FLAG_LOW_LATENCY_ANY = FLAG_LOW_LATENCY | FLAG_LOW_LATENCY_TFM
FLAG_SYMMETRY_AVG = 32
FLAG_SYMMETRY_SLOT = 16384


def labels_dtype() -> np.dtype:
    return np.dtype([("policy", np.float32, (NUM_MOVES,)), ("score_margin", np.float32), ("did_win", np.int32)])


assert labels_dtype().itemsize == 4 * (NUM_MOVES + 2)

NUM_LOSS_TERMS = 19
LOSS_TERMS = ("policy", "policy_aux_dist", "policy_aux_scalar", "outcome", "q6", "q16", "q50", "score_pdf", "score_cdf",
              "own", "gamma_sq", "q_err", "q_score", "q_score_err", "pi_soft", "pi_optimistic", "mcts_dist", "move_hit",
              "outcome_hit")
NUM_V_BUCKETS = 51


def targets_dtype() -> np.dtype:
    f, i = np.float32, np.int32
    return np.dtype([("policy", f, (NUM_MOVES,)), ("policy_aux_dist", f, (NUM_MOVES,)), ("own", f, (361,)),
                     ("mcts_value_dist", f, (NUM_V_BUCKETS,)), ("score_margin", f), ("q6", f), ("q16", f), ("q50", f),
                     ("q6_score", f), ("q16_score", f), ("q50_score", f), ("policy_aux", i), ("has_pi_aux_dist", i),
                     ("has_mcts_value_dist", i)])


assert targets_dtype().itemsize == 4 * 1146 and len(LOSS_TERMS) == NUM_LOSS_TERMS


class EngineError(RuntimeError):
    pass


class Kind(enum.IntEnum):
    kUnknown = 0
    kTrt = 1
    kTF = 2
    kTFTrt = 3
    kTFXla = 4
    kHip = 5


_lib = None


def lib():
    global _lib
# ... 319 lines not shown
    def flops_per_position(self):
        t, c = C.c_double(0), C.c_double(0)
        self._L.p3hip_flops_per_position(self._h, C.byref(t), C.byref(c))
        return t.value, c.value

    def close(self) -> None:
        if getattr(self, "_h", None):
            self._L.p3hip_destroy(self._h)
            self._h = None

    def __del__(self):
        try:
            self.close()
        except Exception:
            pass

    def _ck(self, rc: int, what: str) -> None:
        if rc != 0:
            raise EngineError(f"{what} failed (rc={rc}): " + self._L.p3hip_last_error(self._h).decode())


def aux_outputs(rec) -> dict:
    rec = np.asarray(rec)
    if rec.shape[-1] != AUX_LEN:
        raise ValueError(f"an aux record has {AUX_LEN} floats, not {rec.shape[-1]}")
    return {k: rec[..., a:b] for k, (a, b) in AUX_SEGMENTS.items()}


def debug_plan(path: str, flags: int = 0):
    L = lib()
    n_q, dig = C.c_int(0), C.c_uint64(0)
    name = L.p3hip_debug_plan(path.encode(), flags, C.byref(n_q), C.byref(dig))
    if name is None:
        raise EngineError("p3hip_create: " + L.p3hip_create_error().decode())
    return name.decode(), n_q.value, dig.value


def debug_graph_table(keys, capacity: int = 64):
    L = lib()
    L.p3hip_debug_graph_table.argtypes = [C.c_void_p, C.c_void_p, C.c_int, C.c_int, C.c_void_p, C.c_void_p]
    pairs = [(k, k) if np.isscalar(k) else tuple(k) for k in keys]
    npos = np.array([p[0] for p in pairs], np.int32)
    total = np.array([p[1] for p in pairs], np.int32)
    action = np.full(len(pairs), -1, np.int32)
    evicted = np.full(len(pairs), -2, np.int32)
    if L.p3hip_debug_graph_table(npos.ctypes.data, total.ctypes.data, len(pairs), int(capacity), action.ctypes.data,
                                 evicted.ctypes.data) != 0:
        raise ValueError("p3hip_debug_graph_table: bad argument")
    return action.tolist(), evicted.tolist()


def debug_poison_table() -> dict:
    L = lib()
    L.p3hip_debug_poison_table.restype = C.c_char_p
    L.p3hip_debug_poison_table.argtypes = []
    out = {}
    for line in L.p3hip_debug_poison_table().decode().splitlines():
        name, cls, zero_range = line.split("\t")
        if name in out:
            raise ValueError(f"p3hip_debug_poison_table: {name} has two rows")
        out[name] = (cls, zero_range)
    return out


def debug_tfm_split(npos: int, heads: int, n_cu: int = 256):
    L = lib()
    L.p3hip_debug_tfm_split.argtypes = [C.c_int, C.c_int, C.c_int, C.POINTER(C.c_int), C.POINTER(C.c_int)]
    s, t = C.c_int(0), C.c_int(0)
    if L.p3hip_debug_tfm_split(npos, heads, n_cu, C.byref(s), C.byref(t)) != 0:
        raise ValueError("p3hip_debug_tfm_split: bad argument or bad P3HIP_TFM_SPLIT")
    return s.value, t.value


def debug_edge_split(npos: int, c_pad: int, n_cu: int = 256):
    L = lib()
    L.p3hip_debug_edge_split.argtypes = [C.c_int, C.c_int, C.c_int] + [C.POINTER(C.c_int)] * 3
    s, d, h = C.c_int(0), C.c_int(0), C.c_int(0)
    if L.p3hip_debug_edge_split(npos, c_pad, n_cu, C.byref(s), C.byref(d), C.byref(h)) != 0:
        assert (s.value, d.value, h.value) == (1, 1, 1)
        raise ValueError("p3hip_debug_edge_split: bad argument or bad P3HIP_EDGE_SPLIT")
    return s.value, d.value, h.value


def debug_split(npos: int, kw: int, cout: int, n_cu: int = 256):
    L = lib()
    L.p3hip_debug_split.argtypes = [C.c_int, C.c_int, C.c_int, C.c_int, C.POINTER(C.c_int), C.POINTER(C.c_int)]
    s, t = C.c_int(0), C.c_int(0)
    if L.p3hip_debug_split(npos, kw, cout, n_cu, C.byref(s), C.byref(t)) != 0:
        raise ValueError("p3hip_debug_split: bad argument or bad P3HIP_SPLIT")
    return s.value, t.value


def pack_sconv(w: np.ndarray, cin_pad: int, cout_pad: int) -> np.ndarray:
    w = np.ascontiguousarray(w, np.float32)
    taps, cin, cout = w.shape
    L = lib()
    L.p3hip_debug_pack_sconv.restype = C.c_long
    L.p3hip_debug_pack_sconv.argtypes = [C.c_void_p, C.c_int, C.c_int, C.c_int, C.c_int, C.c_int, C.c_void_p, C.c_long]
    out = np.zeros(taps * cin_pad * cout_pad, np.float16)
    n = L.p3hip_debug_pack_sconv(w.ctypes.data, taps, cin, cout, cin_pad, cout_pad, out.ctypes.data, out.size)
    if n != out.size:
        raise ValueError(f"pack_sconv: the image has {n} elements, expected {out.size}")
    return out.reshape(cout_pad // 16, cin_pad // 32, taps, 64, 8)


def pack_wconv(w: np.ndarray, cin_pad: int, cout_pad: int) -> np.ndarray:
    w = np.ascontiguousarray(w, np.float32)
    taps, cin, cout = w.shape
    if taps != 9:
        raise ValueError("pack_wconv: a 3x3 conv has 9 taps")
    L = lib()
    L.p3hip_debug_pack_wconv.restype = C.c_long
    L.p3hip_debug_pack_wconv.argtypes = [C.c_void_p, C.c_int, C.c_int, C.c_int, C.c_int, C.c_void_p, C.c_long]
    out = np.zeros(16 * cin_pad * cout_pad, np.float16)
    n = L.p3hip_debug_pack_wconv(w.ctypes.data, cin, cout, cin_pad, cout_pad, out.ctypes.data, out.size)
    if n != out.size:
        raise ValueError(f"pack_wconv: the image has {n} elements, expected {out.size}")
    return out.reshape(cout_pad // 16, cin_pad // 32, 16, 64, 8)


def debug_wconv_grid(npos: int, cout: int, n_cu: int = 256, unit: int = -1):
    L = lib()
    L.p3hip_debug_wconv_grid.argtypes = [C.c_int, C.c_int, C.c_int, C.POINTER(C.c_int), C.POINTER(C.c_long), C.c_long,
                                         C.POINTER(C.c_long), C.POINTER(C.c_int), C.POINTER(C.c_int)]
    grid, units, t0, nt, c0 = C.c_int(0), C.c_long(0), C.c_long(0), C.c_int(0), C.c_int(0)
    if unit < 0:
        if L.p3hip_debug_wconv_grid(npos, cout, n_cu, C.byref(grid), C.byref(units), -1, None, None, None) != 0:
            raise ValueError("p3hip_debug_wconv_grid: bad argument")
        return grid.value, units.value
    if L.p3hip_debug_wconv_grid(npos, cout, n_cu, C.byref(grid), C.byref(units), unit, C.byref(t0), C.byref(nt), C.byref(c0)) != 0:
        raise ValueError("p3hip_debug_wconv_grid: bad argument")
    return grid.value, units.value, t0.value, nt.value, c0.value


def rope_table():
    cos = np.zeros((361, 32), np.float64)
    sin = np.zeros((361, 32), np.float64)
    L = lib()
    L.p3hip_rope_table.argtypes = [C.c_void_p, C.c_void_p]
    L.p3hip_rope_table.restype = None
    L.p3hip_rope_table(cos.ctypes.data, sin.ctypes.data)
    return cos, sin


def rope_table_dim(head_dim: int):
    cos = np.zeros((361, head_dim), np.float64)
    sin = np.zeros((361, head_dim), np.float64)
    L = lib()
    L.p3hip_rope_table_dim.argtypes = [C.c_int, C.c_void_p, C.c_void_p]
    L.p3hip_rope_table_dim.restype = C.c_int
    if L.p3hip_rope_table_dim(int(head_dim), cos.ctypes.data, sin.ctypes.data) != 0:
        raise ValueError(f"the engine has no RoPE table of head width {head_dim} (32 or 64)")
    return cos, sin


def symmetry_maps():
    fwd = np.zeros((8, 361), np.uint16)
    inv = np.zeros((8, 361), np.uint16)
    lib().p3hip_symmetry_maps(fwd.ctypes.data, inv.ctypes.data)
    return fwd, inv


def debug_symmetry_rows(masks, rows: int):
    m = np.ascontiguousarray(masks, np.uint8)
    first = np.zeros(max(len(m), 1), np.int32)
    total = C.c_int(0)
# ... 11 lines not shown
```

Measured before the change: 226,500 positions/s.

## Run stem and fused heads kernels as two smaller workgroups per CU

For the fused C=256 path, the stem init kernel now runs with 4 waves per workgroup and 64-channel output passes. Its weight stream is repacked on the host so the halved passes can use a smaller LDS ring, letting two workgroups fit on each CU. The fused heads kernel gets a single-position-group variant that drops the big dense matrices from LDS and reads them from global memory, so two workgroups fit per CU there too. The aim is better latency hiding and CU fill in these edge kernels. The cost is more weight passes, more global reads in the heads dense phase, and an extra device buffer for the repacked stem weights.

```diff
diff --git a/include/p3hip.h b/include/p3hip.h
--- a/include/p3hip.h
+++ b/include/p3hip.h
@@ -163,6 +163,7 @@
 int p3hip_debug_wconv_grid(int npos, int cout, int n_cu, int* grid, long* units, long unit, long* tile0, int* ntiles, int* cout0);
 int p3hip_debug_tfm_split(int npos, int heads, int n_cu, int* parts, int* tokens);
 int p3hip_debug_edge_split(int npos, int c_pad, int n_cu, int* stem, int* dense, int* heads);
+int p3hip_debug_edge_wg_lds(int c, int v, int* stem, int* heads);
 int p3hip_graph_state(const p3hip_engine* e);
 int p3hip_graph_stats(const p3hip_engine* e, uint64_t out[5]);
 int p3hip_debug_graph_table(const int* npos, const int* total, int n, int capacity, int* action, int* evicted);
diff --git a/p3achygo_amd/csrc/engine.cpp b/p3achygo_amd/csrc/engine.cpp
--- a/p3achygo_amd/csrc/engine.cpp
+++ b/p3achygo_amd/csrc/engine.cpp
@@ -86,6 +86,7 @@
 size_t symtab_bytes(const p3hip_engine* e) { return (size_t)e->batch * 5; }
 size_t quant_bytes(const p3hip_engine* e) { return (size_t)e->plan.n_q * 4; }
 size_t arena_bytes(const p3hip_engine* e) { return e->arena_bytes; }
+size_t stem64_bytes(const p3hip_engine* e) { return e->plan.choice.stem_wg2 ? (size_t)e->plan.init_nms * 128 * 128 : 0; }
 size_t cache_entries(const p3hip_engine* e) { return (size_t)e->cache.mask + 1; }
 size_t batch_words(const p3hip_engine* e) { return (size_t)e->batch * 4; }
 
@@ -137,6 +138,7 @@
     {P3_BUF(loss.d_terms), P3_BYTES(batch_words(e) * P3HIP_NUM_LOSS_TERMS), BufClass::Poisoned},
     {P3_BUF(loss.d_sums), P3_BYTES(P3HIP_NUM_LOSS_TERMS * sizeof(double)), BufClass::Poisoned},
     {P3_BUF(d_arena), arena_bytes, BufClass::State},
+    {P3_BUF(d_stem64), stem64_bytes, BufClass::State},
     {P3_BUF(d_amax), quant_bytes, BufClass::State},
     {P3_BUF(d_ascale), quant_bytes, BufClass::State},
     {P3_BUF(cache.d_tkeys), P3_BYTES(cache_entries(e) * 16), BufClass::State},
@@ -316,6 +318,13 @@
                           e->check(hipMemsetAsync(e->d_amax, 0, quant_bytes(e), e->stream), "hipMemset amax") &&
                           e->check(hipMemsetAsync(e->d_ascale, 0, quant_bytes(e), e->stream), "hipMemset scales")));
   if (!ok) return fail(e->err);
+  std::vector<unsigned char> stem64;
+  if (e->plan.choice.stem_wg2) {
+    stem64 = halve_stem_passes(ar.host.data() + e->plan.init_w_off, e->plan.init_nms);
+    if (!e->check(hipMalloc((void**)&e->d_stem64, stem64_bytes(e)), "hipMalloc stem stream") ||
+        !e->check(hipMemcpyAsync(e->d_stem64, stem64.data(), stem64.size(), hipMemcpyHostToDevice, e->stream), "upload stem stream"))
+      return fail(e->err);
+  }
   e->h_scale.assign(e->plan.n_q, 0.0f);
   memset(e->h_feats, 0, B * kFeatBytes);
   if (!e->check(hipMemsetAsync(e->d_feats, 0, feats_bytes(e), e->stream), "hipMemset feats") ||
@@ -353,7 +362,7 @@
   if (!e) return;
   if (e->stream || e->d_arena) (void)hipSetDevice(e->device);
   if (e->stream) hipStreamSynchronize(e->stream);
-  hipFree(e->d_arena); hipFree(e->d_feats); hipFree(e->d_x); hipFree(e->d_t); hipFree(e->d_u); hipFree(e->d_s);
+  hipFree(e->d_arena); hipFree(e->d_stem64); hipFree(e->d_feats); hipFree(e->d_x); hipFree(e->d_t); hipFree(e->d_u); hipFree(e->d_s);
   hipFree(e->d_hp); hipFree(e->d_pool); hipFree(e->d_out); hipFree(e->d_res); hipFree(e->d_qkv);
   hipFree(e->d_sfeats); hipFree(e->d_cout); hipFree(e->d_aux); hipFree(e->d_symtab);
   if (e->h_symtab) hipHostFree(e->h_symtab);
@@ -406,6 +415,13 @@
   if (opt.split_s) { *strips = opt.split_s; *tile = opt.split_t; }
   else p3::sconv_split(npos, kw, cout, n_cu, strips, tile);
   return 0;
+}
+
+int p3hip_debug_edge_wg_lds(int c, int v, int* stem, int* heads) {
+  if (!stem || !heads) return 1;
+  *stem = (int)p3::init_wg2_lds_bytes(c);
+  *heads = (int)p3::headsx_wg2_lds_bytes(c, v);
+  return *stem && *heads ? 0 : 1;
 }
 
 int p3hip_debug_edge_split(int npos, int c_pad, int n_cu, int* stem, int* dense, int* heads) {
diff --git a/p3achygo_amd/csrc/engine.h b/p3achygo_amd/csrc/engine.h
--- a/p3achygo_amd/csrc/engine.h
+++ b/p3achygo_amd/csrc/engine.h
@@ -62,6 +62,7 @@
 
   unsigned char* d_arena = nullptr;
   size_t arena_bytes = 0;
+  unsigned char* d_stem64 = nullptr;
   p3::HeadsArgs heads_args{};
   bool calibrating = false, have_scales = false;
   unsigned* d_amax = nullptr;
diff --git a/p3achygo_amd/csrc/forward.cpp b/p3achygo_amd/csrc/forward.cpp
--- a/p3achygo_amd/csrc/forward.cpp
+++ b/p3achygo_amd/csrc/forward.cpp
@@ -224,6 +224,10 @@
     edge_split_of(e, p.npos, &stem, &dense, &heads);
     if (stem > 1) return e->check(p3::launch_init_split(C, a, stem, e->n_cu, e->stream), "launch k_init_split");
   }
+  if (e->plan.choice.stem_wg2) {
+    a.wstream = e->d_stem64; a.nms_total = 2 * pl.init_nms;
+    return e->check(p3::launch_init(C, a, std::min(p.npos, 2 * e->n_cu), e->stream, true), "launch k_init (two per CU)");
+  }
   return e->check(runs_conv_any(e->plan.choice) ? p3::launch_init_any(C, a, grid_for(e, p.npos, 1), e->stream)
                                              : p3::launch_init(C, a, grid_for(e, p.npos, 1), e->stream), "launch k_init");
 }
@@ -470,7 +474,7 @@
     int stem = 1, dense = 1;
     edge_split_of(e, p.npos, &stem, &dense, &hparts);
   }
-  if (!(e->plan.choice.heads_fused ? e->check(p3::launch_headsx(C, h, e->n_cu, e->stream), "launch k_headsx")
+  if (!(e->plan.choice.heads_fused ? e->check(p3::launch_headsx(C, h, e->n_cu, e->stream, e->plan.choice.heads_wg2), "launch k_headsx")
         : hparts > 1               ? e->check(p3::launch_heads_split(h, e->d_pool, hparts, e->stream), "launch k_heads_pool / points / softmax")
                                    : e->check(p3::launch_heads(h, p.npos, e->stream), "launch k_heads"))) return false;
   if (!aux) return true;
diff --git a/p3achygo_amd/csrc/heads_dense_phase.inc b/p3achygo_amd/csrc/heads_dense_phase.inc
--- a/p3achygo_amd/csrc/heads_dense_phase.inc
+++ b/p3achygo_amd/csrc/heads_dense_phase.inc
@@ -6,12 +6,12 @@
   } else if (t >= 64 && t < 64 + V) {
     const int o = t - 64;
     float s = hl[L::oq_embed_b + o], gm = hl[L::gamma_pre_b + o], b = hl[L::score_pre_b + o];
-#pragma unroll 8
+#pragma unroll kMatUnroll
     for (int k = 0; k < 2 * H; ++k) {
       const float x = sc[L::vp + k];
-      s += x * hl[L::oq_embed_w + k * V + o];
-      gm += x * hl[L::gamma_pre_w + k * V + o];
-      b += x * hl[L::score_pre_w + k * V + o];
+      s += x * w_oq[k * V + o];
+      gm += x * w_gpre[k * V + o];
+      b += x * w_spre[k * V + o];
     }
     sc[L::emb + o] = mish_f(s);
     sc[L::gpre + o] = mish_f(gm);
diff --git a/p3achygo_amd/csrc/kernels.h b/p3achygo_amd/csrc/kernels.h
--- a/p3achygo_amd/csrc/kernels.h
+++ b/p3achygo_amd/csrc/kernels.h
@@ -135,13 +135,15 @@
 
 hipError_t launch_block(int C, int kind, int L, bool wg8, const BlockArgs& a, int n_cu, hipStream_t s);
 int block_macro_step_bytes(int C, bool wg8);
-hipError_t launch_init(int C, const InitArgs& a, int grid, hipStream_t s);
+hipError_t launch_init(int C, const InitArgs& a, int grid, hipStream_t s, bool wg2 = false);
 hipError_t launch_conv1x1(int C, int which, const Conv1x1Args& a, int n_cu, hipStream_t s);
 hipError_t launch_bdense(int C, const BDenseArgs& a, int grid, hipStream_t s);
 hipError_t launch_lconv(int kw, int cin, int cout, const LConvArgs& a, int n_cu, hipStream_t s);
 hipError_t launch_heads(const HeadsArgs& a, int grid, hipStream_t s);
 inline bool heads_fusable(int C, int V) { return (C == 128 || C == 256) && (V == 32 || V == 48 || V == 64); }
-hipError_t launch_headsx(int C, const HeadsArgs& a, int n_cu, hipStream_t s);
+hipError_t launch_headsx(int C, const HeadsArgs& a, int n_cu, hipStream_t s, bool wg2 = false);
+size_t init_wg2_lds_bytes(int C);
+size_t headsx_wg2_lds_bytes(int C, int V);
 
 constexpr int kCacheWays = 8;
 struct CacheKey { unsigned long long lo, hi, sym; };
diff --git a/p3achygo_amd/csrc/kernels.hip b/p3achygo_amd/csrc/kernels.hip
--- a/p3achygo_amd/csrc/kernels.hip
+++ b/p3achygo_amd/csrc/kernels.hip
@@ -308,9 +308,9 @@
   P3_SPAN(7);
 }
 
-template <int C, int CP = 128>
-__global__ void __launch_bounds__(kWG, 2) k_init(InitArgs a) {
-  init_body<CP>(a, FixedW<C>{});
+template <int C, int CP = 128, int NW = 8>
+__global__ void __launch_bounds__(NW * 64, 2) k_init(InitArgs a) {
+  init_body<CP, NW>(a, FixedW<C>{});
 }
 
 template <int CIN, int COUT, bool PRE, int EPI>
@@ -330,13 +330,15 @@
   bdense_body(a, FixedW<C>{});
 }
 
-template <int H, int V>
+template <int H, int V, bool MATS = true>
 struct HeadsLds {
+  static constexpr int mat = MATS ? 2 * H * V : 0;
   static constexpr int gd_w = 0;
   static constexpr int oq_embed_w = gd_w + 2 * H * H;
-  static constexpr int gamma_pre_w = oq_embed_w + 2 * H * V;
-  static constexpr int score_pre_w = gamma_pre_w + 2 * H * V;
-  static constexpr int oq_out_w = score_pre_w + (2 * H + 1) * V;
+  static constexpr int gamma_pre_w = oq_embed_w + mat;
+  static constexpr int score_pre_w = gamma_pre_w + mat;
+  static constexpr int score_row_w = score_pre_w + mat;
+  static constexpr int oq_out_w = score_row_w + V;
   static constexpr int gamma_out_w = oq_out_w + V * 14;
   static constexpr int score_out_w = gamma_out_w + V;
   static constexpr int pass_w = score_out_w + V;
@@ -392,6 +394,8 @@
               score_out_b = a.score_out_b[0];
   float* sc = hl + L::n_weights + g * L::n_scratch;
   const float* base = sc + L::base, * w_sp = hl + L::score_pre_w + (2 * H) * V, * w_so = hl + L::score_out_w;
+  const float* w_oq = hl + L::oq_embed_w, * w_gpre = hl + L::gamma_pre_w, * w_spre = hl + L::score_pre_w;
+  constexpr int kMatUnroll = 8;
   __syncthreads();
 
   for (int pos4 = blockIdx.x * L::kGroups; pos4 < a.npos; pos4 += gridDim.x * L::kGroups) {
@@ -477,36 +481,39 @@
   }
 }
 
-template <int C, int H, int V>
+template <int C, int H, int V, int NG = 2>
 struct HeadsxLds {
-  using L = HeadsLds<H, V>;
-  static constexpr int kGroups = 2, NS = C / 32;
+  using L = HeadsLds<H, V, NG == 2>;
+  static constexpr int kGroups = NG, NS = C / 32;
   static constexpr int part = L::n_weights + kGroups * L::n_scratch;
   static constexpr int n_part = kGroups * 4 * 4 * H;
   static constexpr size_t conv_off = ((size_t)(part + n_part) * 4 + 15) / 16 * 16;
   static constexpr size_t bytes = conv_off + (size_t)6 * NS * 1024;
 };
 
-template <int C, int H, int V>
-__global__ void __launch_bounds__(512, 2) k_headsx(HeadsArgs a) {
-  static_assert(H == 32 && C % 32 == 0, "head channels");
-  using L = HeadsLds<H, V>;
-  using X = HeadsxLds<C, H, V>;
+template <int C, int H, int V, int NG = 2>
+__global__ void __launch_bounds__(NG * 256, 2) k_headsx(HeadsArgs a) {
+  static_assert(H == 32 && C % 32 == 0 && (NG == 1 || NG == 2), "head channels; position groups");
+  using X = HeadsxLds<C, H, V, NG>;
+  using L = typename X::L;
+  using L0 = HeadsLds<H, V>;
   constexpr int NS = X::NS;
   extern __shared__ __attribute__((aligned(16))) float hl[];
-  const int tid = threadIdx.x, g = tid >> 8, t = tid & 255;
+  const int tid = threadIdx.x, g = tid >> 8, t_wg = tid & 255, t = t_wg;
   const int wid = t >> 6, lane = t & 63;
   const int n = lane & 15, q = lane >> 4;
-  static_assert(L::n_weights == heads_image_floats(H, V) && L::n_weights % 4 == 0, "image = HeadsLds");
+  static_assert(L0::n_weights == heads_image_floats(H, V) && L0::n_weights % 4 == 0, "image = HeadsLds");
+  constexpr int kHead = L0::oq_embed_w / 4, kCut = (L0::n_weights - L::n_weights) / 4;
+  static_assert(L0::oq_embed_w % 4 == 0 && L::n_weights % 4 == 0 && L::score_row_w + kCut * 4 == L0::score_row_w, "16-byte pieces");
   {
     const f32x4* src = (const f32x4*)a.image;
     f32x4* dst = (f32x4*)hl;
-    for (int i = tid; i < L::n_weights / 4; i += 512) dst[i] = src[i];
+    for (int i = tid; i < L::n_weights / 4; i += NG * 256) dst[i] = src[i < kHead ? i : i + kCut];
   }
   {
     const f32x4* src = (const f32x4*)a.conv_a;
     f32x4* dst = (f32x4*)((char*)hl + X::conv_off);
-    for (int i = tid; i < 6 * NS * 64; i += 512) dst[i] = src[i];
+    for (int i = tid; i < 6 * NS * 64; i += NG * 256) dst[i] = src[i];
   }
   const float pass_b0 = a.pass_b[0], opt_pass_b = a.opt_pass_b[0], gamma_out_b = a.gamma_out_b[0],
               score_out_b = a.score_out_b[0];
@@ -603,6 +610,8 @@
         }
       }
     __syncthreads();
+    {
+    const int t = NG == 1 ? launder(t_wg) : t_wg, wid = t >> 6, lane = t & 63, n = lane & 15, q = lane >> 4;
     if (t < 4 * H) {
       const int kind = t / H, ch = t - kind * H;
       const float p0 = part[kind * H + ch], p1 = part[4 * H + kind * H + ch], p2 = part[8 * H + kind * H + ch],
@@ -612,6 +621,10 @@
       else dst[H + ch] = fmaxf(fmaxf(p0, p1), fmaxf(p2, p3));
     }
     __syncthreads();
+    const float* __restrict__ w_oq = NG == 2 ? hl + L::oq_embed_w : a.image + L0::oq_embed_w;
+    const float* __restrict__ w_gpre = NG == 2 ? hl + L::gamma_pre_w : a.image + L0::gamma_pre_w;
+    const float* __restrict__ w_spre = NG == 2 ? hl + L::score_pre_w : a.image + L0::score_pre_w;
+    constexpr int kMatUnroll = NG == 2 ? 8 : 16;
 #include "heads_dense_phase.inc"
     {
       float gb[2][4], mw[2][4], omw[2][4];
@@ -658,7 +671,7 @@
         const int z = launder(0);
 #pragma unroll 8
         for (int k = 0; k < V; ++k) {
-          const float b = sc[L::base + z + k], w = hl[L::score_pre_w + (2 * H) * V + z + k], o = hl[L::score_out_w + z + k];
+          const float b = sc[L::base + z + k], w = hl[L::score_row_w + z + k], o = hl[L::score_out_w + z + k];
           acc = __builtin_elementwise_fma(mish_f2(__builtin_elementwise_fma(sv, f32x2{w, w}, f32x2{b, b})), f32x2{o, o}, acc);
         }
         sc[L::logits + s0] = gam * acc[0];
@@ -667,6 +680,7 @@
     }
     __syncthreads();
 #include "heads_softmax_phase.inc"
+    }
   }
 }
 
@@ -712,10 +726,17 @@
   return hipFuncSetAttribute((const void*)kernel, hipFuncAttributeMaxDynamicSharedMemorySize, (int)lds);
 }
 
-hipError_t launch_init(int C, const InitArgs& a, int grid, hipStream_t s) {
+constexpr size_t kInitWg2Lds = Geo<1, 16, 5, 4>::ACT_BYTES + ring_bytes(64) + 256 * 4;
+static_assert(2 * kInitWg2Lds <= 160 * 1024, "k_init<256, 64, 4>: two workgroups per CU");
+size_t init_wg2_lds_bytes(int C) { return C == 256 ? kInitWg2Lds : 0; }
+
+hipError_t launch_init(int C, const InitArgs& a, int grid, hipStream_t s, bool wg2) {
   using G = Geo<1, 16, 5>;
   constexpr size_t lds = G::ACT_BYTES + ring_bytes(128) + 384 * 4;
-  if (C == 192) {
+  if (wg2) {
+    if (C != 256) return hipErrorInvalidValue;
+    hipLaunchKernelGGL((k_init<256, 64, 4>), dim3(grid), dim3(256), kInitWg2Lds, s, a);
+  } else if (C == 192) {
     constexpr size_t lds64 = G::ACT_BYTES + ring_bytes(64) + 192 * 4;
     hipLaunchKernelGGL((k_init<192, 64>), dim3(grid), dim3(kWG), lds64, s, a);
   } else if (C == 384) {
@@ -842,18 +863,31 @@
   return hipGetLastError();
 }
 
-template <int C, int V>
+template <int C, int V, int NG = 2>
 static hipError_t launch_headsx_t(const HeadsArgs& a, int n_cu, hipStream_t s) {
-  using X = HeadsxLds<C, 32, V>;
-  static_assert(X::bytes <= 160 * 1024, "LDS");
+  using X = HeadsxLds<C, 32, V, NG>;
+  constexpr int per_cu = 3 - NG;
+  static_assert(per_cu * X::bytes <= 160 * 1024, "LDS");
   static AttrOnce once;
-  if (hipError_t e = ensure_lds(once, k_headsx<C, 32, V>, X::bytes); e != hipSuccess) return e;
-  const int groups = (a.npos + X::kGroups - 1) / X::kGroups;
-  hipLaunchKernelGGL((k_headsx<C, 32, V>), dim3(groups < n_cu ? groups : n_cu), dim3(512), X::bytes, s, a);
-  return hipGetLastError();
-}
-
-hipError_t launch_headsx(int C, const HeadsArgs& a, int n_cu, hipStream_t s) {
+  if (hipError_t e = ensure_lds(once, k_headsx<C, 32, V, NG>, X::bytes); e != hipSuccess) return e;
+  const int groups = (a.npos + X::kGroups - 1) / X::kGroups, cap = per_cu * n_cu;
+  hipLaunchKernelGGL((k_headsx<C, 32, V, NG>), dim3(groups < cap ? groups : cap), dim3(NG * 256), X::bytes, s, a);
+  return hipGetLastError();
+}
+
+size_t headsx_wg2_lds_bytes(int C, int V) {
+  if (C != 256) return 0;
+  return V == 64 ? HeadsxLds<256, 32, 64, 1>::bytes : V == 48 ? HeadsxLds<256, 32, 48, 1>::bytes
+       : V == 32 ? HeadsxLds<256, 32, 32, 1>::bytes : 0;
+}
+
+hipError_t launch_headsx(int C, const HeadsArgs& a, int n_cu, hipStream_t s, bool wg2) {
+  if (wg2) {
+    if (C == 256 && a.V == 64) return launch_headsx_t<256, 64, 1>(a, n_cu, s);
+    if (C == 256 && a.V == 48) return launch_headsx_t<256, 48, 1>(a, n_cu, s);
+    if (C == 256 && a.V == 32) return launch_headsx_t<256, 32, 1>(a, n_cu, s);
+    return hipErrorInvalidValue;
+  }
   if (C == 256 && a.V == 64) return launch_headsx_t<256, 64>(a, n_cu, s);
   if (C == 256 && a.V == 48) return launch_headsx_t<256, 48>(a, n_cu, s);
   if (C == 256 && a.V == 32) return launch_headsx_t<256, 32>(a, n_cu, s);
diff --git a/p3achygo_amd/csrc/layer_kernels.h b/p3achygo_amd/csrc/layer_kernels.h
--- a/p3achygo_amd/csrc/layer_kernels.h
+++ b/p3achygo_amd/csrc/layer_kernels.h
@@ -59,29 +59,28 @@
   for (int i = threadIdx.x; i < C; i += kWG) { dst[384 + i] = scale[i]; dst[384 + C + i] = shift[i]; }
 }
 
-template <int CP, class W>
+template <int CP, int NW = 8, class W>
 __device__ __forceinline__ void init_body(InitArgs a, W wc) {
   const int C = wc.get();
-  using G = Geo<1, 16, 5>;
-  if constexpr (W::fixed) static_assert(W::get() % CP == 0, "output passes");
+  using G = Geo<1, 16, 5, NW>;
+  if constexpr (W::fixed) static_assert(W::get() % CP == 0 && W::get() <= NW * 64, "output passes; one thread per channel of the game-state dense");
   using T = Tiling<G, CP>;
   extern __shared__ __attribute__((aligned(16))) char smem[];
   constexpr uint32_t kRingOff = G::ACT_BYTES;
   act_zero<G>(smem);
-  Ring<T::RS> ring;
+  Ring<T::RS, NW> ring;
   ring_init(ring, smem, a.wstream, a.nms_total, kRingOff);
   lds_barrier();
   const int lane = threadIdx.x & 63;
   const int wid = __builtin_amdgcn_readfirstlane(threadIdx.x >> 6);
   const int lg = wid / T::CG;
-  const int lr = lane & 31, h = lane >> 5;
 
   for (int pos = blockIdx.x; pos < a.npos; pos += gridDim.x) {
 #include "stem_planes.inc"
 
     float* bias_lds = (float*)(smem + kRingOff + ring_bytes(CP));
     int tc = threadIdx.x;
-    if constexpr (!W::fixed) tc = launder(tc);
+    if constexpr (!W::fixed || NW == 4) tc = launder(tc);
     if (tc < C) {
       float b = a.game_b[tc];
 #pragma unroll
@@ -90,11 +89,13 @@
     }
 
 #pragma unroll 1
-    for (int cp = 0; cp < C / CP; ++cp) {
+    for (int pass = 0; pass < C / CP; ++pass) {
       f32x16 acc[2][T::NT];
       acc_zero<G, CP>(acc);
       conv_segment<G, CP, 5, 28>(ring, smem, acc);
-      const int bias_cp = cp;
+      const int ln = NW == 4 ? launder(lane) : lane, cp = NW == 4 ? launder(pass) : pass;
+      const int lr = ln & 31, h = ln >> 5;
+      const int bias_cp = pass;
 #include "stem_epilogue.inc"
     }
     lds_barrier();
diff --git a/p3achygo_amd/csrc/plan.cpp b/p3achygo_amd/csrc/plan.cpp
--- a/p3achygo_amd/csrc/plan.cpp
+++ b/p3achygo_amd/csrc/plan.cpp
@@ -3,6 +3,7 @@
 #include <cmath>
 #include <cstdio>
 #include <cstdlib>
+#include <cstring>
 #include <utility>
 
 #include "../../include/p3hip.h"
@@ -27,6 +28,7 @@
   o.bcast_fuse = !set("P3HIP_NO_BFUSE");
   o.dense_fuse = !set("P3HIP_NO_DFUSE");
   o.heads_fuse = !set("P3HIP_NO_HFUSE");
+  o.edge_wg2 = !set("P3HIP_EDGE_WG1");
   o.stop_block = num("P3HIP_DEBUG_STOP_BLOCK", -1);
   o.fuse = !set("P3HIP_NO_FUSE");
   o.join = o.fuse && !set("P3HIP_NO_JOIN");
@@ -319,8 +321,10 @@
   c.any_width = (c.path == Path::Int8Conv3 || c.path == Path::Winograd3) && (tr == Trunk::OtherConv || opt.conv_any);
   c.CB = is_layerwise(c.path) ? p3::conv_any_slice(C) : (is_tfm(c.path) ? 128 : Cb);
   c.CPI = is_layerwise(c.path) ? p3::conv_any_init_pass(C) : 128;
+  c.stem_wg2 = opt.edge_wg2 && c.path == Path::Fused && C == 256;
   c.heads_image = !is_f32(c.path) && p3::heads_fusable(C, wf.V);
   c.heads_fused = c.heads_image && opt.heads_fuse && !runs_conv_any(c);
+  c.heads_wg2 = c.stem_wg2 && c.heads_fused;
   if (is_tfm(c.path)) {
     c.tfm_heads = Cb;
     c.tfm_D = wf.model_C / Cb;
@@ -865,6 +869,19 @@
     }
 }
 
+std::vector<unsigned char> halve_stem_passes(const unsigned char* s128, int nms) {
+  constexpr size_t row = 64 * 8 * 2, blk128 = 4 * row;
+  constexpr int nblk = 28;
+  const int npass = nms * 4 / nblk;
+  std::vector<unsigned char> out((size_t)nms * 4 * blk128);
+  unsigned char* dst = out.data();
+  for (int p = 0; p < 2 * npass; ++p)
+    for (int k = 0; k < nblk; ++k)
+      for (int h = 0; h < 2; ++h, dst += row)
+        memcpy(dst, s128 + ((size_t)(p / 2) * nblk + k) * blk128 + (size_t)(2 * h + p % 2) * row, row);
+  return out;
+}
+
 bool build_plan(const WeightFile& wf, uint32_t flags, const Options& opt, Plan& plan, Arena& ar, std::string& err) {
   plan.choice = choose_plan(wf, flags, opt, err);
   const Path path = plan.choice.path;
diff --git a/p3achygo_amd/csrc/plan.h b/p3achygo_amd/csrc/plan.h
--- a/p3achygo_amd/csrc/plan.h
+++ b/p3achygo_amd/csrc/plan.h
@@ -19,6 +19,7 @@
   bool bcast_fuse = true;
   bool dense_fuse = true;
   bool heads_fuse = true;
+  bool edge_wg2 = true;
   int stop_block = -1;
   bool fuse = true, join = true;
   int stagger = -1;
@@ -73,6 +74,7 @@
   int CPI = 0;
   bool heads_image = false;
   bool heads_fused = false;
+  bool stem_wg2 = false, heads_wg2 = false;
   int tfm_heads = 0, tfm_D = 0;
   bool any_width = false;
 };
@@ -172,6 +174,8 @@
 
 bool build_plan(const WeightFile& wf, uint32_t flags, const Options& opt, Plan& plan, Arena& ar, std::string& err);
 
+std::vector<unsigned char> halve_stem_passes(const unsigned char* s128, int nms);
+
 void spiral_rope_table(int D, double* cos_out, double* sin_out);
 
 }
diff --git a/p3achygo_amd/csrc/stem_planes.inc b/p3achygo_amd/csrc/stem_planes.inc
--- a/p3achygo_amd/csrc/stem_planes.inc
+++ b/p3achygo_amd/csrc/stem_planes.inc
@@ -1,6 +1,6 @@
   const unsigned char* f = (const unsigned char*)a.feats + (size_t)pos * FeatOff::size;
   const int color = (signed char)f[FeatOff::color];
-  for (int loc = threadIdx.x; loc < kNLoc; loc += kWG) {
+  for (int loc = threadIdx.x; loc < kNLoc; loc += G::NW * 64) {
     h8 lo = {0, 0, 0, 0, 0, 0, 0, 0}, hi = {0, 0, 0, 0, 0, 0, 0, 0};
     auto our = [&](int off) {
       return (_Float16)((signed char)f[off + loc] == color ? 1.0f : 0.0f);
diff --git a/p3achygo_amd/engine.py b/p3achygo_amd/engine.py
--- a/p3achygo_amd/engine.py
+++ b/p3achygo_amd/engine.py
@@ -28,7 +28,7 @@
     "p3hip_debug_split", "p3hip_debug_pack_sconv", "p3hip_debug_tfm_split", "p3hip_debug_edge_split",
     "p3hip_debug_poison", "p3hip_debug_poison_table",
     "p3hip_debug_pack_wconv", "p3hip_debug_wconv_grid",
-    "p3hip_graph_stats", "p3hip_debug_graph_table",
+    "p3hip_graph_stats", "p3hip_debug_graph_table", "p3hip_debug_edge_wg_lds",
 ]
 
 FLAG_RUN_ALL_SLOTS = 2
@@ -514,6 +514,15 @@
     return s.value, d.value, h.value
 
 
+def debug_edge_wg_lds(c: int, v: int):
+    L = lib()
+    L.p3hip_debug_edge_wg_lds.argtypes = [C.c_int, C.c_int] + [C.POINTER(C.c_int)] * 2
+    s, h = C.c_int(0), C.c_int(0)
+    if L.p3hip_debug_edge_wg_lds(c, v, C.byref(s), C.byref(h)) != 0:
+        raise ValueError("p3hip_debug_edge_wg_lds: no two-to-a-CU form for C = %d, V = %d" % (c, v))
+    return s.value, h.value
+
+
 def debug_split(npos: int, kw: int, cout: int, n_cu: int = 256):
     L = lib()
     L.p3hip_debug_split.argtypes = [C.c_int, C.c_int, C.c_int, C.c_int, C.POINTER(C.c_int), C.POINTER(C.c_int)]
```

Result: no change. 228,000 positions/s (median of 3 runs) (+0.7%).
